# JvanKatwijk/sdr-j-fm

Measured on AMD Instinct MI355X. Metric: IQ MSamples/s demodulated to 48 kHz stereo, higher is better.
Workload: dtype f32 (stage A: 3-term split-f16 MFMA with a per-tile block exponent, f32 accumulate); 1 GPU; config4; population=established, channels_per_gpu=4096, channels_total=4096, streams_per_gpu=4096, block_samples_per_channel=230400, parallelism=channels sharded, 1 rank/GPU

## Files before the change

sdr-j-fm_amd/csrc/fmx_api.hip:

```cpp
#include "fmx_host.h"
#include "fmx_fftconv.h"
#include "fmx_design.h"

#include <cmath>
#include <cstdio>
#include <cstdlib>
#include <cstring>

thread_local std::string fmx::host::g_err;

namespace {

int env_int(const char *name, int dflt) { const char *v = getenv(name); return v ? atoi(v) : dflt; }
struct EnvSwitches {
    bool pieces_serial;
    bool tail_split;
};
const EnvSwitches &env_switches() {
    static const EnvSwitches sw{env_int("FMX_CALL_PIECES_SERIAL", 0) != 0, env_int("FMX_TAIL_SPLIT", 1) != 0};
    return sw;
}

int next_pow2(int64_t v) { int64_t p = 1; while (p < v) p <<= 1; return (int)p; }

int build_front_set(int32_t bw, int32_t inputRate, int32_t fmRate, int decim, int p, float *taps , FrontSet *fs) {
    std::vector<double> g(1, 1.0);
    double S1 = 0.0, S2 = 0.0;
    if (decim > 1) {
        const int32_t IRate = inputRate / 6;
        design::DecimKernel k1 = design::decim(4 * inputRate / IRate + 1, fmRate / 2, inputRate);
        design::DecimKernel k2 = design::decim(IRate / fmRate + 1, fmRate / 2, IRate);
        const int D1 = inputRate / IRate;
        g.assign((size_t)(D1 * (k2.hn.size() - 1) + k1.hn.size()), 0.0);
        for (size_t i = 0; i < k2.hn.size(); i++)
            for (size_t l = 0; l < k1.hn.size(); l++) g[D1 * i + l] += (double)k2.hn[i] * (double)k1.hn[l];
        S1 = k1.sum; S2 = k2.sum;
    }
    int L = 0;
    if (bw > 0) {
        std::vector<float> hin = design::lowpass(251, bw / 2, inputRate);
        g = design::convolve(g, design::to_double(hin));
        L = 2 * 32768 - 251;
    }
    const int NT = (int)g.size();
    const int64_t e = (int64_t)decim * p + decim - 1 - L;
    int64_t delay = -(e >= 0 ? e / 12 : -((-e + 11) / 12));
    const int off = (int)(e + 12 * delay);
    fs->off = off; fs->delay_fm = (int32_t)delay; fs->zshift = 0;
    int nd = 0;
    std::fill(taps, taps + A_TAPS_STRIDE, 0.f);
    for (int d = 0; d < A_MAX_ND; d++)
        for (int r = 0; r < DECIM; r++) {
            const int k = 12 * d + off - r;
            if (k >= 0 && k < NT) { taps[(d + 1) * DECIM + r] = (float)g[k]; nd = d + 1; }
        }
    fs->nd = nd;
    fs->gain_re = (float)(1.0 - S1 * S2); fs->gain_im = (float)(S1 + S2);
    double hs = 0, mk = 0;
    for (int d = 0; d < A_MAX_ND; d++)
        for (int r = 0; r < DECIM; r++) {
            const double v = (double)taps[(d + 1) * DECIM + r];
            hs += v; mk += v * (double)(12 * d + off - r);
        }
    fs->hsum = (float)hs;
    const double q0 = (double)off - mk / hs + 1.0;
    const int K = -(int)std::floor(q0 / 12.0);
    fs->dc_k = K; fs->dc_w = (float)((q0 + 12.0 * K) / 12.0);
    return (int)delay;
}

void build_audio_set(int32_t lf, int32_t fmRate, const std::vector<float> &rs, float *taps , AudioSet *as) {
    std::vector<double> g = design::to_double(rs);
    as->delay = 0;
    if (lf > 0) {
        std::vector<float> ha = design::lowpass(AUDIO_TAPS, lf, fmRate);
        g = design::convolve(design::to_double(ha), g);
        as->delay = AUDIO_DELAY;
    }
    as->ntaps = (int)g.size();
    std::fill(taps, taps + C_TAPS_STRIDE, 0.f);
    for (int kk = 0; kk < as->ntaps; kk++) taps[kk] = (float)g[as->ntaps - 1 - kk];
}

}

int fmx::host::ensure_sets(fmx_handle h) {
    std::vector<int32_t> fk, ak;
    for (int c = 0; c < h->channels; c++) {
        int32_t b = h->user[c].bw_applied, l = h->user[c].lf_applied > 0 ? h->user[c].lf_applied : 0;
        if (h->ola_mode) { b = 0; l = 0; }
        auto it = std::find(fk.begin(), fk.end(), b);
        if (it == fk.end()) { fk.push_back(b); it = fk.end() - 1; }
        h->params[c].front_set = (int)(it - fk.begin()) * h->twins;
        auto ia = std::find(ak.begin(), ak.end(), l);
        if (ia == ak.end()) { ak.push_back(l); ia = ak.end() - 1; }
        h->params[c].audio_set = (int)(ia - ak.begin());
    }
    if (fk != h->front_keys) {
        h->front_keys = fk;
        const size_t TW = (size_t)h->twins, NS = fk.size() * TW;
        h->h_front_taps.assign(NS * A_TAPS_STRIDE, 0.f);
        h->h_front_sets.resize(NS);
        for (size_t i = 0; i < fk.size(); i++) {
            int dmin = 0x7fffffff;
            std::vector<int> dl(TW);
            for (size_t p = 0; p < TW; p++) {
                dl[p] = build_front_set(fk[i], h->cfg.inputRate, h->cfg.fmRate, h->decim, (int)p, &h->h_front_taps[(i * TW + p) * A_TAPS_STRIDE], &h->h_front_sets[i * TW + p]);
                dmin = std::min(dmin, dl[p]);
            }
            for (size_t p = 0; p < TW; p++) { h->h_front_sets[i * TW + p].zshift = dl[p] - dmin; h->h_front_sets[i * TW + p].delay_fm = (int32_t)(TW * (size_t)dmin); }
        }
        if ((int)NS > h->front_cap) {
            h->mem.release(h->d_front_taps); h->mem.release(h->d_front_sets);
            h->front_cap = std::max<int>((int)NS, 4);
            FMXCHK(h->mem.alloc(h->d_front_taps, (size_t)A_TAPS_DEV * h->front_cap));
            FMXCHK(h->mem.alloc(h->d_front_sets, (size_t)h->front_cap));
        }
        HIPCHK(hipDeviceSynchronize());
        std::vector<float> dev(NS * A_TAPS_DEV, 0.f);
        for (size_t i = 0; i < NS; i++)
            for (int d = 0; d < A_MAX_ND; d++)
                for (int r = 0; r < DECIM; r++)
                    dev[i * A_TAPS_DEV + r * A_TAPS_ROW + d] = h->h_front_taps[i * A_TAPS_STRIDE + (d + 1) * DECIM + r];
        HIPCHK(hipMemcpy(h->d_front_taps, dev.data(), sizeof(float) * dev.size(), hipMemcpyHostToDevice));
        HIPCHK(hipMemcpy(h->d_front_sets, h->h_front_sets.data(), sizeof(FrontSet) * NS, hipMemcpyHostToDevice));
        h->T.front_taps = h->d_front_taps; h->T.front_sets = h->d_front_sets;
    }
    if (ak != h->audio_keys) {
        h->audio_keys = ak;
        h->h_audio_taps.assign(ak.size() * C_TAPS_STRIDE, 0.f);
        h->h_audio_sets.resize(ak.size());
        for (size_t i = 0; i < ak.size(); i++)
            build_audio_set(ak[i], h->cfg.fmRate, h->h_rs_taps, &h->h_audio_taps[i * C_TAPS_STRIDE], &h->h_audio_sets[i]);
        if ((int)ak.size() > h->audio_cap) {
            h->mem.release(h->d_audio_taps); h->mem.release(h->d_audio_sets);
            h->audio_cap = std::max<int>((int)ak.size(), 4);
            FMXCHK(h->mem.alloc(h->d_audio_taps, (size_t)C_TAPS_STRIDE * h->audio_cap));
            FMXCHK(h->mem.alloc(h->d_audio_sets, (size_t)h->audio_cap));
        }
        HIPCHK(hipDeviceSynchronize());
        HIPCHK(hipMemcpy(h->d_audio_taps, h->h_audio_taps.data(), sizeof(float) * h->h_audio_taps.size(), hipMemcpyHostToDevice));
        HIPCHK(hipMemcpy(h->d_audio_sets, h->h_audio_sets.data(), sizeof(AudioSet) * ak.size(), hipMemcpyHostToDevice));
        h->T.audio_taps = h->d_audio_taps; h->T.audio_sets = h->d_audio_sets;
        {
            std::vector<float> lp(ak.size() * AUDIO_TAPS, 0.f);
            for (size_t i = 0; i < ak.size(); i++) if (ak[i] > 0) { const std::vector<float> ha = design::lowpass(AUDIO_TAPS, ak[i], h->cfg.fmRate); std::copy(ha.begin(), ha.end(), lp.begin() + i * AUDIO_TAPS); }
            h->mem.release(h->T.audio_lp_taps);
            FMXCHK(h->mem.upload(h->T.audio_lp_taps, lp));
            if (!h->T.rs_taps) FMXCHK(h->mem.upload(h->T.rs_taps, h->h_rs_taps));
            std::vector<float2> W(fftc::W_COUNT), spec(ak.size() * 4 * fftc::N);
            fftc::make_twiddles(W.data());
            for (size_t i = 0; i < ak.size(); i++) {
                const int nt = h->h_audio_sets[i].ntaps;
                const float *rev = &h->h_audio_taps[i * C_TAPS_STRIDE];
                for (int p = 0; p < 4; p++) {
                    std::vector<float> gp;
                    for (int kk = p; kk < nt; kk += 4) gp.push_back(rev[nt - 1 - kk]);
                    fftc::make_spectrum(gp.data(), (int)gp.size(), &spec[(i * 4 + p) * fftc::N], W.data());
                }
            }
            h->mem.release(h->T.audio_spec);
            FMXCHK(h->mem.upload(h->T.audio_spec, spec));
        }
    }
    h->sets_dirty = false;
    return FMX_OK;
}

namespace {

void refresh_derived(fmx_handle h, int c) {
    const ChanUser &u = h->user[c];
    ChanParams &p = h->params[c];
    const int32_t fmRate = h->cfg.fmRate;
    if (u.deemph_us >= 1) {
        const float Tau = (float)(1000000.0 / u.deemph_us);
        p.deemph_alpha = (float)(1.0 / ((double)((float)fmRate / Tau) + 1.0));
    } else {
        p.deemph_alpha = (float)(1.0 / (fmRate / (1000000.0 / 50.0 + 1)));
    }
    p.deemph_l2 = (float)std::log2((double)(1.0f - p.deemph_alpha));
    p.volume = u.ctor_volume ? 0.5f : std::pow(10.0f, u.volume_db / 20.0f);
    p.left_ch = (u.balance > 0 ? (float)((100 - u.balance) / 100.0) : 1.0f);
    p.right_ch = (u.balance < 0 ? (float)((100 + u.balance) / 100.0) : 1.0f);
    p.panorama = (float)(int16_t)u.panorama / 100.0f;
}

int ensure_lo_table(fmx_handle h) {
    if (h->T.lo_table) return FMX_OK;
    const int32_t R = h->cfg.inputRate;
    std::vector<float2> tab((size_t)R);
    for (int32_t i = 0; i < R; i++)
        tab[i] = make_float2((float)std::cos(2.0 * design::kPi * i / R), (float)std::sin(2.0 * design::kPi * i / R));
    return h->mem.upload(h->T.lo_table, tab);
}

int ensure_rds_body(fmx_handle h);
int ensure_rds(fmx_handle h) {
    if (h->rds_alloc) return FMX_OK;
    const int rc = ensure_rds_body(h);
    if (rc) { h->rds_mem.release_all(); h->R = RdsBuffers{}; h->d_rds_nc0 = nullptr; h->rds_stage = nullptr; }
    return rc;
}
int ensure_rds_body(fmx_handle h) {
    const size_t C = (size_t)h->channels;
    const int32_t fmRate = h->cfg.fmRate;
    DevMem &M = h->rds_mem;
    RdsBuffers &R = h->R;
    FMXCHK(M.alloc(R.in_blk, C * RDS_BLK, true));
    FMXCHK(M.alloc(R.bpreal, C * 2 * RDS_BLK, true));
    FMXCHK(M.alloc(R.bp_over, 2 * C * 768, true));
    FMXCHK(M.alloc(R.hil, C * 2 * RDS_BLK, true));
    FMXCHK(M.alloc(R.hil_over, 2 * C * 768, true));
    FMXCHK(M.alloc(R.phase_ring, C * RDS_PHASE_RING, true));
    FMXCHK(M.alloc(R.U, C * 32768));
    FMXCHK(M.alloc(R.V, C * 32768));
    FMXCHK(M.alloc(R.rds24, C * RDS24_RING, true));
    R.pitch = h->pitch;
    FMXCHK(M.alloc(R.mf, (size_t)(h->work_nj / 8 + 8) * h->pitch));
    R.mfc_stride = ((h->work_nj / 8 + 8 + 2 + 7) / 8) * 8;
    FMXCHK(M.alloc(R.mfc, (size_t)R.mfc_stride * C, true));
    FMXCHK(M.alloc(R.mfm, (size_t)R.mfc_stride * C, true));
    FMXCHK(M.alloc(R.bits, C * RDS_BITS_CAP, true));
    FMXCHK(M.alloc(R.sym, C * RDS_SYM_CAP, true));
    {
        RdsState s0; std::memset(&s0, 0, sizeof(s0));
        s0.gain = 9.0f; s0.mu = 0.f; s0.skip = 3; s0.sample_count = 0;
        s0.c_limit = (float)(2 * design::kPi * (double)10.0f / (double)(float)24000);
        std::vector<RdsState> init(C, s0);
        FMXCHK(M.upload(R.state, init));
    }
    {
        const int N = 32768, D = 768;
        std::vector<float> k = design::bandpass(D, 3 * 19000 - 4800 / 2, 3 * 19000 + 4800 / 2, fmRate);
        std::vector<float2> S((size_t)N), Hm((size_t)N);
        std::vector<double> cs((size_t)N), sn((size_t)N);
        for (int i = 0; i < N; i++) { cs[i] = std::cos(-2 * design::kPi * i / N); sn[i] = std::sin(-2 * design::kPi * i / N); }
        for (int f = 0; f < N; f++) {
            double re = 0, im = 0;
            for (int i = 0; i < D; i++) {
                const int a = (int)(((int64_t)f * i) & (N - 1));
                re += (double)k[2 * i] * cs[a] - (double)k[2 * i + 1] * sn[a];
                im += (double)k[2 * i] * sn[a] + (double)k[2 * i + 1] * cs[a];
            }
            S[f] = make_float2((float)re, (float)im);
            Hm[f] = make_float2(f == 0 || f == N / 2 ? 1.0f : (f < N / 2 ? 2.0f : 0.0f), 0.f);
        }
        FMXCHK(M.upload(R.S_bp, S));
        FMXCHK(M.upload(R.S_hil, Hm));
        {
            std::vector<float2> Sr((size_t)N);
            for (int f = 0; f < N; f++) {
                const float2 a = S[(size_t)f], b = S[(size_t)((N - f) & (N - 1))];
                Sr[(size_t)f] = make_float2(0.5f * (a.x + b.x), 0.5f * (a.y - b.y));
            }
            FMXCHK(M.upload(R.S_bp_re, Sr));
        }
        std::vector<float> dk = design::decim_complex(11, 24000 / 2, fmRate);
        std::vector<float> rr = design::rrc(1.0, 24000, 2 * 1187.5f, 1.0, 45);
        float2 *dd;
        FMXCHK(M.alloc(dd, 11));
        FMXCHK(M.upload(R.rrc, rr));
        HIPCHK(hipMemcpy(dd, dk.data(), sizeof(float2) * 11, hipMemcpyHostToDevice));
        R.dec_taps = dd;
    }
    {
        FMXCHK(M.alloc(R.c_ring, C * RDS24_RING, true));
        FMXCHK(M.alloc(R.f_ring, C * RDS24_RING, true));
        FMXCHK(M.alloc(R.state1, C, true));
        std::vector<float> co = design::lowpass(RDS1_FIR, 2 * 2400, 24000);
        const std::vector<float> mk = design::rds1_match_kernel(24000);
        if ((int)mk.size() != RDS1_MATCH) return fail(FMX_E_HIP, "unexpected length of the RDS_1 matched filter");
        co.insert(co.end(), mk.begin(), mk.end());
        const design::Iir bp = design::iir_butterworth_bandpass(7, (int32_t)(1187.5 - 6), (int32_t)(1187.5 + 6), 24000);
        if (bp.nq != RDS1_QUADS) return fail(FMX_E_HIP, "unexpected biquad count of the RDS_1 band-pass");
        for (int i = 0; i < RDS1_QUADS; i++) { co.push_back(bp.q[i][1]); co.push_back(bp.q[i][2]); co.push_back(bp.q[i][4]); co.push_back(bp.q[i][5]); }
        co.push_back(bp.gain);
        FMXCHK(M.upload(R.rds1_coef, co));
        h->h_rds1 = co;
    }
    {
        FMXCHK(M.alloc(R.state3, C, true));
        std::vector<float2> sc24(24000);
        for (int i = 0; i < 24000; i++) sc24[i] = make_float2((float)std::cos(2 * design::kPi * i / 24000), (float)std::sin(2 * design::kPi * i / 24000));
        FMXCHK(M.upload(R.sincos24, sc24));
    }
    FMXCHK(M.alloc(R.sync, C, true));
    FMXCHK(M.alloc(R.groups, C * RDS_GROUP_RING, true));
    if (!h->ev_call) HIPCHK(hipEventCreateWithFlags(&h->ev_call, hipEventDisableTiming));
    h->rd.bits.assign(C, 0);
    {
        FMXCHK(M.alloc(h->d_rds_nc0, C, true));
        FMXCHK(M.alloc(R.chlist, C, true));
        R.nc0 = h->d_rds_nc0;
        h->rds_nc.assign(C, 0); h->rds_nc0.assign(C, -1); h->last_m0.assign(C, 0); h->last_m1.assign(C, 0);
    }
    h->rds_alloc = true;
    return FMX_OK;
}

int ola_alloc_side(fmx_handle h, fmx_handle_s::OlaSide &S, int L, int degree) {
    const size_t C = (size_t)h->channels;
    S.L = L; S.degree = degree;
    FMXCHK(h->mem.alloc(S.A, C * L, true));
    FMXCHK(h->mem.alloc(S.C, C * L, true));
    FMXCHK(h->mem.alloc(S.over, C * OLA_MAX_TAPS, true));
    FMXCHK(h->mem.alloc(S.over_new, C * OLA_MAX_TAPS, true));
    FMXCHK(h->mem.alloc(S.taps, C * OLA_MAX_TAPS, true));
    S.inp.assign(C, 0); S.on.assign(C, 0); S.key.assign(C, -1);
    return FMX_OK;
}
int ensure_ola(fmx_handle h) {
    if (h->d_v) return FMX_OK;
    const size_t C = (size_t)h->channels;
    FMXCHK(h->mem.alloc(h->d_v, C * h->cfg.max_block));
    FMXCHK(h->mem.alloc(h->d_u, C * h->cfg.max_block));
    FMXCHK(h->mem.alloc(h->d2ring, C * h->dring, true));
    h->pre_look.max_tiles = (int32_t)(h->cfg.max_block / PRE_TILE_SAMPLES + 1);
    FMXCHK(h->mem.alloc(h->pre_look.maps, C * h->pre_look.max_tiles));
    FMXCHK(h->mem.alloc(h->pre_look.flags, C * h->pre_look.max_tiles, true));
    FMXCHK(h->mem.alloc(h->pre_look.tickets, C, true));
    h->pre_look.ticket_base = 0;
// ... 352 lines not shown
    if (nd.prepass) { const int rc = ensure_prepass_arrays(h); if (rc) return rc; }
    for (int c = 0; c < h->channels; c++) {
        ChanUser &u = h->user[c];
        if (u.squelch_value != u.squelch_old) {
            u.squelch_level = u.squelch_value; u.squelch_old = u.squelch_value;
            const SquelchThr t = squelch_thresholds(u.squelch_level);
            h->params[c].squelch_thr = t.level; h->params[c].squelch_nthr = t.noise;
            h->params_dirty = true;
        }
    }
    if (h->params_dirty) {
        HIPCHK(hipDeviceSynchronize());
        HIPCHK(hipMemcpy(h->d_params, h->params.data(), sizeof(ChanParams) * h->channels, hipMemcpyHostToDevice));
        h->act_up.resize((size_t)h->channels);
        for (int c = 0; c < h->channels; c++) h->act_up[(size_t)c] = h->params[(size_t)c].actions;
        h->params_dirty = false;
    }
    return FMX_OK;
}

void actions_consumed(fmx_handle h, bool had_fm_samples) {
    std::lock_guard<std::mutex> lk(h->mtx);
    if (h->act_up.size() != (size_t)h->channels) return;
    const int32_t done = ACT_DC_RESET | (had_fm_samples ? (ACT_TRIGGER_FREQ | ACT_RESTART_PSS) : 0);
    for (int c = 0; c < h->channels; c++) {
        const int32_t clr = h->act_up[(size_t)c] & done;
        if (clr) { h->params[(size_t)c].actions &= ~clr; h->act_up[(size_t)c] &= ~clr; h->params_dirty = true; }
    }
}

void frames_geom(const fmx_handle h, int64_t n, CallGeom *G) {
    G->g0 = h->g_total; G->n = n;
    G->J0 = h->g_total / h->decim; G->J1 = (h->g_total + n) / h->decim;
    G->M0 = 48 * (G->J0 / 192); G->M1 = 48 * (G->J1 / 192);
}
int64_t call_frames(const fmx_handle h, int64_t n) { CallGeom G{}; frames_geom(h, n, &G); return conv2_out(h, G.M1) - conv2_out(h, G.M0); }

int ensure_pipe_streams(fmx_handle h) {
    if (h->pipe_sA) return FMX_OK;
    int lo = 0, hi = 0;
    HIPCHK(hipDeviceGetStreamPriorityRange(&lo, &hi));
    HIPCHK(hipStreamCreateWithPriority(&h->pipe_sA, hipStreamNonBlocking, lo));
    HIPCHK(hipStreamCreateWithPriority(&h->pipe_sB, hipStreamNonBlocking, lo));
    HIPCHK(hipStreamCreateWithPriority(&h->pipe_sP, hipStreamNonBlocking, hi));
    for (hipEvent_t *e : {&h->pipe_ev0, &h->pipe_evA, &h->pipe_evD, &h->pipe_evP, &h->pipe_evE, &h->pipe_evB[0], &h->pipe_evB[1]}) HIPCHK(hipEventCreateWithFlags(e, hipEventDisableTiming));
    return FMX_OK;
}

int check_call(fmx_handle h, int32_t fmt, float s16_den, int64_t n, int64_t pcm_stride) {
    if (const ParamCheck pc = check_iq_format(fmt, s16_den); pc.code) return fail(pc.code, pc.msg);
    if (n <= 0 || n > h->cfg.max_block) return fail(FMX_E_TOO_LARGE, "n_complex must be in [1, max_block]");
    if (call_frames(h, n) > pcm_stride) return fail(FMX_E_TOO_LARGE, "pcm_stride smaller than the frames this call produces");
    return FMX_OK;
}

struct CallArgs { int32_t fmt; float s16_den; int64_t stream_stride, pcm_stride; };

int promotion_turn(fmx_handle h, bool head, hipStream_t s, bool *capture) {
    bool do_promote = false, do_demote = false;
    {
        std::lock_guard<std::mutex> lk(h->mtx);
        if (h->ola_mode) {
            const bool ok = demotable(h);
            if (!ok || h->promo_recapture) { h->demo_capture = false; h->promo_have = 0; }
            else if (!h->demo_capture) { h->demo_capture = true; h->promo_have = 0; *capture = true; }
            else if (h->promo_have >= DEMO_TAIL_IN && head) do_demote = true;
            else *capture = true;
            h->promo_recapture = false;
        }
        else if (!h->promo_pending) h->promo_recapture = false;
        else if (h->promo_recapture) { h->promo_recapture = false; h->promo_have = 0; }
        else if (h->promo_have >= PROMO_TAIL_IN && head) do_promote = true;
        else *capture = true;
    }
    if (do_promote) return promote(h, s);
    if (do_demote) return demote(h, s);
    return FMX_OK;
}

int capture_samples(fmx_handle h, const void *d_iq, const CallArgs &a, const CallGeom &G, hipStream_t sa) {
    if (h->tail_iq && h->promo_have + G.n > h->tail_cap) return FMX_OK;
    if (!h->tail_iq) {
        h->tail_cap = PROMO_TAIL_IN + h->cfg.max_block;
        FMXCHK(h->mem.alloc(h->tail_iq, (size_t)h->streams * h->tail_cap));
        FMXCHK(h->mem.alloc(h->tail_snap, (size_t)h->channels));
    }
    if (h->promo_have == 0) { h->promo_g0 = h->g_total; launch_promo_state(h->B.state, h->tail_snap, h->channels, 0, sa); FMX_LAUNCHED(); }
    launch_capture(d_iq, a.fmt, G.iq_scale, a.stream_stride, G.n, h->streams, h->tail_iq, h->tail_cap, h->promo_have, sa); FMX_LAUNCHED();
    h->promo_have += G.n;
    return FMX_OK;
}

int stage_a(fmx_handle h, CallGeom &G, const void *d_iq, hipStream_t s, hipStream_t sa) {
    const FrontParts fp = plan_front_parts(G.g0, G.n, h->front_parts.load(), h->twins, h->channels, h->n_cus);
    if (fp.parts > 1 && !h->B.fsnap) {
        const size_t C = (size_t)h->channels;
        h->B.dc_pitch = (int32_t)(h->cfg.max_block / FRONT_TILE + 2);
        FMXCHK(h->mem.alloc(h->B.dc_tiles, 2 * (size_t)h->streams * h->B.dc_pitch));
        FMXCHK(h->mem.alloc(h->B.fsnap, C));
        FMXCHK(h->mem.alloc(h->B.hist_snap, C * DECIM * A_HIST_COLS));
        FMXCHK(h->mem.alloc(h->B.dcv_snap, C * DCV_SAVE));
    }
    const FrontChoice fc = choose_front(h->needs.front4_ok, h->needs.any_lo, h->front_kernel.load(), fp.parts, h->channels, h->n_cus);
    G.parts = fc.parts; G.part_tiles = fp.part_tiles; G.front4 = fc.front4;
    h->last_front_kernel = (G.front4 && front4_tiles(G, d_iq) > 0) ? 3 : 1;
    if (h->ola_mode) {
        if (const int rc = ola_input_side(h, G, h->B, d_iq, s)) return rc;
        CallGeom Gp = G; Gp.pre_processed = 1; Gp.iq_format = 0; Gp.iq_scale = 1.0f; Gp.stream_stride = h->cfg.max_block; Gp.streams_private = h->twins == 1 ? 1 : 0;
        launch_front(h->T, h->B, Gp, h->d_u, h->channels, s);
    } else
    launch_front(h->T, h->B, G, d_iq, h->channels, sa);
    FMX_LAUNCHED();
    return FMX_OK;
}

int stage_b(fmx_handle h, const CallGeom &G, int k, bool piped, int second, hipStream_t s, hipStream_t sa) {
    if (piped) {
        HIPCHK(hipEventRecord(h->pipe_evA, sa)); HIPCHK(hipStreamWaitEvent(s, h->pipe_evA, 0));
        if (k >= 2) HIPCHK(hipStreamWaitEvent(sa, h->pipe_evB[k & 1], 0));
        DeviceBuffers Bk = h->B;
        if (k & 1) { const size_t off = (size_t)prepass_half(h->work_nj) * (size_t)h->pitch; Bk.w_iq += off; Bk.w_osc += off; }
        const PrepassStreams ps{sa, h->pipe_sP, h->pipe_evD, h->pipe_evP};
        launch_demod_fused(h->T, Bk, G, h->channels, s, &ps);
        HIPCHK(hipEventRecord(h->pipe_evB[k & 1], s));
    } else if (second > 0) {
        HIPCHK(hipEventRecord(h->pipe_evA, s)); HIPCHK(hipStreamWaitEvent(h->pipe_sA, h->pipe_evA, 0));
        CallGeom G1 = G, G2 = G;
        G1.ch0 = 0; G1.ch_count = h->channels - second; G2.ch0 = h->channels - second; G2.ch_count = second;
        launch_demod_fused(h->T, h->B, G1, h->channels, s);
        launch_demod_fused(h->T, h->B, G2, h->channels, h->pipe_sA);
    } else
    launch_demod_fused(h->T, h->B, G, h->channels, s);
    if (G.J1 > G.J0) {
        int cnt = h->my_count_host + (int)(G.J1 - G.J0);
        if (cnt > (SINCOS_N >> 1)) cnt -= (SINCOS_N >> 1) + 1;
        h->my_count_host = cnt;
    }
    return FMX_OK;
}

int stage_rds(fmx_handle h, const CallGeom &G, hipStream_t s) {
    const int64_t nj = G.J1 - G.J0;
    int modes = 0;
    for (int c = 0; c < h->channels; c++) {
        const int m = h->call_rds_mode[(size_t)c];
        modes |= 1 << m;
        h->rds_nc0[(size_t)c] = m != 0 ? h->rds_nc[(size_t)c] : -1;
    }
    HIPCHK(hipMemcpyAsync(h->d_rds_nc0, h->rds_nc0.data(), sizeof(int64_t) * (size_t)h->channels, hipMemcpyHostToDevice, s));
    launch_rds(h->B, h->R, G, h->channels, h->rds_nc0.data(), modes, s);
    for (int c = 0; c < h->channels; c++) {
        const int64_t a = h->rds_nc0[(size_t)c];
        if (a < 0) { h->last_m0[(size_t)c] = h->last_m1[(size_t)c]; continue; }
        h->last_m0[(size_t)c] = a / 8; h->last_m1[(size_t)c] = (a + nj) / 8;
        h->rds_nc[(size_t)c] = a + nj;
    }
    return FMX_OK;
}

int stage_scan(fmx_handle h, const CallGeom &G, hipStream_t sa) {
    const int64_t nj = G.J1 - G.J0;
    const size_t n = h->call_scan.size();
    h->scan_jobs.resize(n);
    {
        std::lock_guard<std::mutex> lk(h->mtx);
        for (size_t i = 0; i < n; i++) {
            const int c = h->call_scan[i];
            const ScanProduce sp = scan_produce(h->scan_fill[(size_t)c], h->scan_blocks[(size_t)c], nj, G.J0, scan::N, scan::RING);
            h->scan_jobs[i] = ScanJob{c, sp.job_fill, sp.job_slot0, 0};
            for (int64_t b = sp.b0; b < sp.nblk; b++) {
                const size_t slot = (size_t)c * scan::RING + (size_t)sp.slot(b);
                h->scan_end[slot] = sp.end_sample(b);
                h->scan_rec_thr[slot] = h->call_scan_thr[i];
            }
            h->scan_blocks[(size_t)c] = sp.new_blocks;
            h->scan_fill[(size_t)c] = sp.new_fill;
        }
    }
    HIPCHK(hipMemcpyAsync(h->d_scan_jobs, h->scan_jobs.data(), sizeof(ScanJob) * n, hipMemcpyHostToDevice, sa));
    ScanArgs A{};
    A.jobs = h->d_scan_jobs; A.zring = h->B.zring; A.params = h->d_params; A.front_sets = h->d_front_sets; A.W = h->d_scan_W;
    A.carry = h->d_scan_carry; A.rec = h->d_scan_rec; A.J0 = G.J0; A.J1 = G.J1; A.ring_mask = G.ring_mask;
    launch_scan(A, (int)n, sa); FMX_LAUNCHED();
    return FMX_OK;
}

int stage_meter(fmx_handle h, const CallGeom &G, hipStream_t s) {
    const int64_t nj = G.J1 - G.J0;
    if (nj > h->work_nj) return fail(FMX_E_TOO_LARGE, "the piece has more fm samples than stage B's rows hold");
    h->meter_jobs.clear();
    {
        std::lock_guard<std::mutex> lk(h->mtx);
        for (int c = 0; c < h->channels; c++) {
            if (!h->call_meter[(size_t)c]) { h->meter_on_from[(size_t)c] = -1; continue; }
            if (h->meter_on_from[(size_t)c] < 0) h->meter_on_from[(size_t)c] = G.J0;
            const meter::Produce mp = meter::meter_produce(h->meter_on_from[(size_t)c], G.J0, nj, h->meter_produced[(size_t)c]);
            if (mp.first >= G.J1) continue;
            h->meter_jobs.push_back(MeterJob{c, (int32_t)(mp.first - G.J0), (int32_t)mp.slot(0), 0});
            h->meter_produced[(size_t)c] = mp.new_produced;
        }
    }
    const size_t n = h->meter_jobs.size();
    if (n == 0) return FMX_OK;
    HIPCHK(hipMemcpyAsync(h->d_meter_jobs, h->meter_jobs.data(), sizeof(MeterJob) * n, hipMemcpyHostToDevice, s));
    MeterArgs A{};
    A.jobs = h->d_meter_jobs; A.w_dem = h->B.w_dem; A.w_cur = h->B.w_cur; A.state = h->d_meter_state; A.ring = h->d_meter_ring;
    A.J0 = G.J0; A.J1 = G.J1; A.lin_rows = h->B.lin_rows;
    launch_meter(A, (int)n, s); FMX_LAUNCHED();
    return FMX_OK;
}

int stage_scan_mute(fmx_handle h, float2 *d_pcm, int64_t pcm_stride, int64_t frames, hipStream_t s) {
    const size_t n = h->call_scan.size();
    HIPCHK(hipMemcpyAsync(h->d_scan_mute, h->call_scan.data(), sizeof(int32_t) * n, hipMemcpyHostToDevice, s));
    launch_scan_mute(h->d_scan_mute, (int)n, d_pcm, pcm_stride, frames, s); FMX_LAUNCHED();
    return FMX_OK;
}

int stage_audio_meter(fmx_handle h, const CallGeom &G, const float2 *d_pcm, int64_t frames, hipStream_t s) {
    h->loud_jobs.clear();
    {
        std::lock_guard<std::mutex> lk(h->mtx);
        for (int c = 0; c < h->channels; c++) {
            if (!h->call_loud[(size_t)c]) { h->loud_on_from[(size_t)c] = -1; continue; }
            if (h->loud_on_from[(size_t)c] < 0) h->loud_on_from[(size_t)c] = G.M0;
            const loud::Produce ap = loud::audio_produce(h->loud_on_from[(size_t)c], G.M0, frames, h->loud_produced[(size_t)c]);
            h->loud_jobs.push_back(LoudJob{c, ap.first == G.M0 ? 1 : 0, (int32_t)ap.slot(0), ap.reset ? 1 : 0});
            h->loud_produced[(size_t)c] = ap.new_produced;
        }
    }
    const size_t n = h->loud_jobs.size();
    if (n == 0) return FMX_OK;
    HIPCHK(hipMemcpyAsync(h->d_loud_jobs, h->loud_jobs.data(), sizeof(LoudJob) * n, hipMemcpyHostToDevice, s));
    LoudArgs A{};
    A.jobs = h->d_loud_jobs; A.pcm = d_pcm; A.pcm_stride = G.pcm_stride; A.state = h->d_loud_state; A.ring = h->d_loud_ring;
    A.M0 = G.M0; A.frames = (int32_t)frames;
    launch_loud(A, (int)n, s); FMX_LAUNCHED();
    return FMX_OK;
}

int stage_c(fmx_handle h, CallGeom &G, float2 *d_pcm, int64_t frames, int second, hipStream_t s) {
    DeviceBuffers Bq = h->B;
    if (h->ola_mode && G.J1 > G.J0) {
        OlaBuffers O{}; O.src = h->B.dring; O.dst = h->d2ring; O.src_stride = O.dst_stride = h->dring; O.src_mask = O.dst_mask = h->dring - 1;
        O.src_pos = O.dst_pos = G.J0;
        HStep st1;
        if (ola_single_step(h, h->ola_au, G.J1 - G.J0, &st1)) {
            OlaStepRef ref; const int rc = step_ref(h, st1, s, &ref); if (rc) return rc;
            ola_fill(h->ola_au, O);
            launch_deemph(h->B, G, h->d2ring, h->channels, s, &ref, &O); FMX_LAUNCHED();
            ola_finish_single(h, h->ola_au, st1, ref, O, s);
        } else {
            const int rc = run_ola(h, h->ola_au, O, G.J1 - G.J0, s); if (rc) return rc;
            launch_deemph(h->B, G, h->d2ring, h->channels, s, nullptr, nullptr); FMX_LAUNCHED();
        }
    }
    if (h->ola_mode) Bq.dring = h->d2ring;
    if (h->gain_pending && G.M1 > G.M0) { G.gain_fix = 1; launch_gain_fix(h->T, Bq, G, h->channels, s); FMX_LAUNCHED(); h->gain_pending = false; }
    if (second > 0) {
        CallGeom G1 = G, G2 = G;
        G1.ch0 = 0; G2.ch0 = h->channels - second;
        launch_audio(h->T, Bq, G1, d_pcm, h->channels - second, s);
        launch_audio(h->T, Bq, G2, d_pcm, second, h->pipe_sA);
        HIPCHK(hipEventRecord(h->pipe_evE, h->pipe_sA)); HIPCHK(hipStreamWaitEvent(s, h->pipe_evE, 0));
    } else if (!h->cv_nt) launch_audio(h->T, Bq, G, d_pcm, h->channels, s);
    else {
        CallGeom G48 = G; G48.pcm_stride = h->x48_stride;
        launch_audio(h->T, Bq, G48, h->d_x48 + h->cv_nt, h->channels, s);
        launch_conv2(h->d_x48, h->x48_stride, h->d_cv_taps, h->cv_p, h->cv_q, h->cv_nt, G.M0, G.M1 - G.M0, conv2_out(h, G.M0), frames,
                     d_pcm, G.pcm_stride, h->channels, s);
    }
    return FMX_OK;
}

int run_piece(fmx_handle h, const CallArgs &a, const void *d_iq, int64_t n, float2 *d_pcm, hipStream_t s, int k, bool overlapped, int64_t *n_frames) {
    bool capture = false;
    int rc = promotion_turn(h, k == 0, s, &capture);
    if (rc || (rc = flush_mailbox(h))) return rc;
    CallGeom G{};
    frames_geom(h, n, &G);
    G.ring_mask = h->ring - 1; G.dring_mask = h->dring - 1; G.sring_mask = h->sring - 1;
    G.input_rate = h->cfg.inputRate; G.pitch = h->pitch; G.streams_private = (h->streams_private && h->twins == 1) ? 1 : 0; G.twins = h->twins; G.channels = h->channels; G.stream_stride = a.stream_stride; G.pcm_stride = a.pcm_stride;
    G.iq_format = a.fmt; G.iq_scale = (a.fmt == 3) ? 1.0f / a.s16_den : 1.0f / 128.0f; G.n_cus = h->n_cus; G.streams = h->streams;
    const int64_t frames = conv2_out(h, G.M1) - conv2_out(h, G.M0);
    const bool rds_running = h->rds_alloc && h->needs.any_rds;
    if (rds_running && G.J1 - G.J0 > RDS_BLK)
        return fail(FMX_E_TOO_LARGE, "with RDS on, a call may cover at most 32000 fm samples (384000 input samples)");
    const bool piped = overlapped && !h->ola_mode && !env_switches().pieces_serial;
    hipStream_t sa = piped ? h->pipe_sA : s;
    G.host_count1 = piped ? h->my_count_host + 1 : 0;
    ProfRec pr{}; const bool prof = h->prof_on;
    if (prof) {
        for (int i = 0; i < 4; i++) HIPCHK(hipEventCreate(&pr.e[i]));
        pr.in_samples = n * h->streams; pr.ch_samples = n * h->channels;
        HIPCHK(hipEventRecord(pr.e[0], sa));
    }
    g_launch_err = hipSuccess;
    h->B.lin_rows = (int32_t)h->work_nj;
    if (capture && (rc = capture_samples(h, d_iq, a, G, sa))) return rc;
    if ((rc = stage_a(h, G, d_iq, s, sa))) return rc;
    if (!h->call_scan.empty() && G.J1 > G.J0 && (rc = stage_scan(h, G, sa))) return rc;
    if (prof) HIPCHK(hipEventRecord(pr.e[1], sa));
    G.stageb_form = h->stageb_form.load(); G.no_deemph = h->ola_mode ? 1 : 0;
    const bool plain = plain_batch(PieceFlags{piped, h->ola_mode, h->B.w_iq != nullptr, h->cv_nt != 0, h->needs.rows_on, rds_running, h->gain_pending, G.stageb_form,
                                              G.J1 > G.J0, G.M1 > G.M0});
    const int second = env_switches().tail_split && plain ? second_group_channels(h->channels, h->n_cus) : 0;
    if (second > 0 && (rc = ensure_pipe_streams(h))) return rc;
    h->last_second_group = second;
    if ((rc = stage_b(h, G, k, piped, second, s, sa))) return rc;
    if (rds_running && (rc = stage_rds(h, G, s))) return rc;
    if (h->meter_alloc && G.J1 > G.J0 && (rc = stage_meter(h, G, s))) return rc;
    if (prof) HIPCHK(hipEventRecord(pr.e[2], s));
    if ((rc = stage_c(h, G, d_pcm, frames, second, s))) return rc;
    if (!h->call_scan.empty() && frames > 0 && (rc = stage_scan_mute(h, d_pcm, G.pcm_stride, frames, s))) return rc;
    if (h->loud_alloc && frames > 0 && (rc = stage_audio_meter(h, G, d_pcm, frames, s))) return rc;
    if (prof) { HIPCHK(hipEventRecord(pr.e[3], s)); h->prof.push_back(pr); }
    FMX_LAUNCHED();
    HIPCHK(g_launch_err);
    actions_consumed(h, G.J1 > G.J0);
    h->last_J0 = G.J0; h->last_J1 = G.J1;
    h->g_total += n;
    if (n_frames) *n_frames = frames;
    return FMX_OK;
}

int run_call(fmx_handle h, const void *d_iq, int32_t fmt, float s16_den, int64_t stream_stride, int64_t n, float2 *d_pcm,
             int64_t pcm_stride, int64_t *n_frames, hipStream_t s) {
    h->last_pieces = 1;
    int rc = check_call(h, fmt, s16_den, n, pcm_stride);
    if (rc) return rc;
    CallShape cs{};
    {
        std::lock_guard<std::mutex> lk(h->mtx);
        const CallNeeds nd = summarize(h);
        cs.any_rds = nd.any_rds; cs.prepass = nd.prepass; cs.pllc = nd.pllc; cs.am = nd.am;
    }
    if (!cs.any_rds && cs.prepass && !h->ola_mode && (rc = ensure_prepass_arrays(h))) return rc;
    cs.n = n; cs.decim = h->decim; cs.call_pieces = h->pipe_rows.load(); cs.channels = h->channels; cs.ola_mode = h->ola_mode; cs.conv2 = h->cv_nt != 0;
    cs.prepass_arrays = h->B.w_iq != nullptr; cs.half = prepass_half(h->work_nj);
    const CallPlan plan = plan_call(cs);
    const bool overlapped = plan.kind == CallKind::OVERLAPPED;
    hipStream_t ps = s;
    if (overlapped) {
        if ((rc = ensure_pipe_streams(h))) return rc;
        HIPCHK(hipEventRecord(h->pipe_ev0, s));
        HIPCHK(hipStreamWaitEvent(h->pipe_sA, h->pipe_ev0, 0)); HIPCHK(hipStreamWaitEvent(h->pipe_sB, h->pipe_ev0, 0));
        ps = h->pipe_sB;
    }
    const CallArgs a{fmt, s16_den, stream_stride, pcm_stride};
    const int64_t bps = bytes_per_sample(fmt);
    int64_t pos = 0, total = 0;
    for (size_t k = 0; k < plan.lens.size(); k++) {
        int64_t got = 0;
        rc = run_piece(h, a, reinterpret_cast<const char *>(d_iq) + pos * bps, plan.lens[k], d_pcm + total, ps, (int)k, overlapped, &got);
        if (rc) { if (overlapped) (void)hipDeviceSynchronize(); return rc; }
        pos += plan.lens[k]; total += got;
    }
    if (overlapped) {
        HIPCHK(hipEventRecord(h->pipe_evE, h->pipe_sB)); HIPCHK(hipStreamWaitEvent(s, h->pipe_evE, 0));
        h->last_pieces = (int)plan.lens.size();
    }
    if (h->rds_alloc) { HIPCHK(hipEventRecord(h->ev_call, s)); h->ev_call_set = true; }
    if (n_frames) *n_frames = total;
    return FMX_OK;
}


}

namespace {

struct Conv2Design { int p = 1, q = 1, nt = 0; std::vector<float> taps; };

int validate_config(const fmx_config *cfg, int *decim_out, Conv2Design *cv) {
    if (cfg->struct_size != (int32_t)sizeof(fmx_config)) return fail(FMX_E_INVALID, "fmx_config.struct_size mismatch");
    if (cfg->channels < 1) return fail(FMX_E_INVALID, "channels must be >= 1");
    if (cfg->fmRate != 192000 || cfg->workingRate != 48000)
        return fail(FMX_E_UNSUPPORTED, "this build implements fmRate 192000 / workingRate 48000 (radio.cpp:68,231-233)");
    int decim = DECIM;
    {
        if (cfg->inputRate < 1 || cfg->inputRate > 100000000) return fail(FMX_E_INVALID, "inputRate out of range");
        if (cfg->inputRate / cfg->fmRate <= 1) decim = 1;
        else {
            const int32_t IRate = cfg->inputRate / 6;
            const int64_t d2 = IRate / cfg->fmRate;
            if ((d2 != 1 && d2 != 2) || 4 * (int64_t)cfg->inputRate / IRate + 1 != 25 || cfg->inputRate / IRate != 6)
                return fail(FMX_E_UNSUPPORTED, "inputRate: built are the rates the reference decimates by 12 (2304000 <= inputRate < 3456000), by 6 "
                                               "(1152000 <= inputRate < 2304000) and not at all (inputRate < 384000); below 1152000 the reference's "
                                               "second decimator has one tap and a zero gain (fir-filters.cpp:327-347), from 3456000 on it divides by 3+");
            decim = 6 * (int)d2;
        }
    }
    *decim_out = decim;
    if (cfg->audioRate != cfg->workingRate) {
        if (cfg->audioRate < 8000 || cfg->audioRate > 192000 ||
            !design::design_conv2(cfg->workingRate, cfg->audioRate, &cv->p, &cv->q, &cv->nt, &cv->taps))
            return fail(FMX_E_UNSUPPORTED, "audioRate: 8000 .. 192000 with audioRate / gcd (audioRate, workingRate) <= 640 (the second converter's phases)");
    }
    if (cfg->max_block < 12 || cfg->max_block > (1 << 20)) return fail(FMX_E_INVALID, "max_block must be in [12, 1048576]");
    int ndev = 0;
    if (hipGetDeviceCount(&ndev) != hipSuccess || ndev <= 0)
        return fail(FMX_E_NO_DEVICE, "no HIP device visible: libfmx has no CPU fallback");
    if (cfg->device < 0 || cfg->device >= ndev) return fail(FMX_E_INVALID, "device ordinal out of range");
    return FMX_OK;
}

int init_channels(fmx_handle h, const fmx_config *cfg, int decim, const Conv2Design &cv) {
    h->cfg = *cfg; h->cfg.stream_of_channel = nullptr;
    h->decim = decim; h->twins = DECIM / decim;
    h->channels = cfg->channels;
    h->streams = cfg->streams > 0 ? cfg->streams : cfg->channels;
    if (cv.nt) {
        h->cv_p = cv.p; h->cv_q = cv.q; h->cv_nt = cv.nt;
        h->x48_stride = cv.nt + cfg->max_block / (4 * h->decim) + 96;
    }
    h->ola_mode = filter_form(0, h->channels).ola_mode;
    h->user.assign(h->channels, ChanUser());
    h->rd.init((size_t)h->channels);
    h->params.assign(h->channels, ChanParams());
    for (int c = 0; c < h->channels; c++) {
        ChanParams &p = h->params[c];
        std::memset(&p, 0, sizeof(p));
        int s = cfg->stream_of_channel ? cfg->stream_of_channel[c] : (cfg->streams > 0 ? c % h->streams : c);
        if (s < 0 || s >= h->streams) return fail(FMX_E_INVALID, "stream_of_channel entry out of range");
        p.stream = s;
        p.fm_mode = 0; p.sound_sel = 0; p.decoder = 3; p.auto_mono = 1; p.pss_active = 1; p.dc_remove = 1;
        p.rds_mode = 0; p.lo_freq = 0; p.lo_period = 0; p.att_l = 1.f; p.att_r = 1.f;
        p.pll_seq = pll_seq(0, h->channels);
        const SquelchThr t = squelch_thresholds(1);
        p.squelch_mode = 0; p.squelch_thr = t.level; p.squelch_nthr = t.noise;
        refresh_derived(h, c);
    }
    std::vector<int> users((size_t)h->streams, 0);
    h->streams_private = true;
    for (auto &p : h->params) if (++users[(size_t)p.stream] > 1) h->streams_private = false;
    return FMX_OK;
}

int init_device(fmx_handle h) {
    hipDeviceProp_t dp;
    HIPCHK(hipGetDeviceProperties(&dp, h->cfg.device));
    h->n_cus = dp.multiProcessorCount;
    int optin = 0;
    if (hipDeviceGetAttribute(&optin, hipDeviceAttributeMaxSharedMemoryPerBlock, h->cfg.device) != hipSuccess) optin = 0;
    h->lds_per_block = std::max((size_t)dp.sharedMemPerBlock, (size_t)optin);
    HIPCHK(hipStreamCreateWithFlags(&h->stream, hipStreamNonBlocking));
    HIPCHK(hipEventCreateWithFlags(&h->ev_in, hipEventDisableTiming));
    return FMX_OK;
}

int build_trig_tables(fmx_handle h) {
    const int32_t fmRate = h->cfg.fmRate;
    std::vector<float2> sc((size_t)SINCOS_N);
    for (int i = 0; i < SINCOS_N; i++)
        sc[i] = make_float2((float)std::cos(2 * design::kPi * i / fmRate), (float)std::sin(2 * design::kPi * i / fmRate));
    FMXCHK(h->mem.upload(h->T.sincos, sc));
    {
        SinPoly sp{}; sp.step = 2 * design::kPi / fmRate;
        bool fits = (fmRate == SINCOS_N);
        for (int i = 0; fits && i < SINCOS_N; i++) {
            float sn, cs;
            sincos_poly(i, sp.step, &sn, &cs);
            if (std::memcmp(&sn, &sc[i].y, 4) != 0) { if (sp.ns < 4) { sp.s_idx[sp.ns] = i; sp.s_val[sp.ns] = sc[i].y; sp.ns++; } else fits = false; }
            if (std::memcmp(&cs, &sc[i].x, 4) != 0) { if (sp.nc < 4) { sp.c_idx[sp.nc] = i; sp.c_val[sp.nc] = sc[i].x; sp.nc++; } else fits = false; }
        }
        sp.ok = fits ? 1 : 0;
        h->T.sp = sp;
    }
    {
        std::vector<double2> tr((size_t)TRIG2_N);
        for (int a = 0; a < TRIG2_A; a++) { double t = 2 * design::kPi * (256.0 * a) / fmRate; tr[a] = make_double2(std::cos(t), std::sin(t)); }
        for (int a = 0; a < TRIG2_APAD; a++) tr[TRIG2_A + a] = tr[a];
        for (int b = 0; b < TRIG2_B; b++) { double t = 2 * design::kPi * (double)b / fmRate; tr[TRIG2_A + TRIG2_APAD + b] = make_double2(std::cos(t), std::sin(t)); }
        bool exact = (fmRate == TRIG2_A * TRIG2_B);
        for (int i = 0; exact && i < SINCOS_N; i++) {
            const double2 ea = tr[i >> 8], eb = tr[TRIG2_A + TRIG2_APAD + (i & 255)];
            const float sn = (float)(ea.y * eb.x + ea.x * eb.y);
            if (std::memcmp(&sn, &sc[i].y, 4) != 0) exact = false;
        }
        if (exact) FMXCHK(h->mem.upload(h->T.trig2, tr));
    }
    {
        const float P32 = 6.2831855f;
        const float C32 = (float)((double)P32 - 2 * design::kPi);
        bool ok = true;
        for (float v = P32; ok && v < P32 + 0.7f; v = std::nextafterf(v, 100.f)) {
            const float want = (float)((double)v - 2 * design::kPi);
            volatile float d = v - P32;
            const float got = d + C32;
            if (std::memcmp(&want, &got, 4) != 0) ok = false;
        }
        h->T.wrap32_c = C32; h->T.wrap32_ok = ok ? 1 : 0;
    }
    std::vector<float> at((size_t)ATAN_N + 1);
    const float St = (float)design::kPi;
    for (int i = 0; i <= ATAN_N; i++) { float f = (float)i / ATAN_N; at[i] = (float)((double)(std::atan(f) * St) / design::kPi); }
    FMXCHK(h->mem.upload(h->T.atan_ppy, at));
    std::vector<float> as((size_t)ARCSINE_N + 1);
    for (int i = 0; i <= ARCSINE_N; i++) as[i] = (float)(std::asin(2.0 * i / ARCSINE_N - 1.0) / 2.0);
    return h->mem.upload(h->T.arcsine, as);
}

int build_filter_tables(fmx_handle h) {
    const int32_t fmRate = h->cfg.fmRate;
    h->h_pss_taps = design::lowpass(PSS_TAPS, 15000, fmRate);
    FMXCHK(h->mem.upload(h->T.pss_taps, h->h_pss_taps));
    h->h_rs_taps = design::resampler(RS_TAPS);
    {
        std::vector<float2> W(fftc::W_COUNT), Hs(fftc::N);
        fftc::make_twiddles(W.data());
        fftc::make_spectrum(h->h_pss_taps.data(), PSS_TAPS, Hs.data(), W.data());
        FMXCHK(h->mem.upload(h->T.fft_w, W));
        FMXCHK(h->mem.upload(h->T.pss_hs, Hs));
    }
    h->T.sincos_C = fmRate / (2 * design::kPi);
    {
        const float F_G = (float)(0.65 * fmRate / 2), Delta_F = (float)(0.95 * fmRate / 2);
        const float B_FM = 2 * (Delta_F + F_G);
        h->T.K_FM = (float)((double)(2 * B_FM) * design::kPi / (double)F_G);
        const float max_dev = (float)(0.95 * (0.5 * fmRate));
        const float fac = (float)(2.0 * design::kPi / fmRate);
        h->T.pll_beta = (float)std::exp(-2.0 * design::kPi * (double)(float)(0.85 * fmRate) / 2 / fmRate);
        h->T.pll_lo = -max_dev * fac; h->T.pll_hi = max_dev * fac; h->T.pll_center = (float)(0 * 2 * design::kPi / fmRate);
    }
    h->T.pil_omega = (float)((double)((float)19000 / (float)fmRate) * (2 * design::kPi));
    h->T.pil_gain = (float)(10 * (2 * design::kPi) / fmRate);
    h->T.K_FM_rcp = 1.0f / h->T.K_FM; h->T.pil_omega_rcp = 1.0f / h->T.pil_omega;
    h->T.pss_alpha = 10.0f / (float)fmRate;
    h->T.pss_lock_alpha = 1.0f / fmRate;
    h->T.afc_l2 = (float)std::log2((double)(1 - 0.0001f));
    h->T.lock_l2 = (float)std::log2(1.0 - (double)(1.0f / 3000.0f));
    h->T.pssmean_l2 = (float)std::log2((double)(1.0f - h->T.pss_lock_alpha));
    return FMX_OK;
}

int alloc_channel_buffers(fmx_handle h, const Conv2Design &cv) {
    DevMem &M = h->mem;
    DeviceBuffers &B = h->B;
    const int32_t max_block = h->cfg.max_block;
    const int64_t fm_per_call = max_block / h->decim + 2;
    h->ring = next_pow2((2 * 32768 - 251) / h->decim + 1 + fm_per_call + 512);
    h->dring = next_pow2(std::max<int64_t>(AUDIO_DELAY + C_MAX_TAPS, h->channels > OLA_MAX_CH ? PROMO_TAIL_AU + 8 : 0) + fm_per_call + 192 + 4 * C_TILE);
    h->sring = 4096;
    const size_t C = (size_t)h->channels;
    const size_t CT = C * (size_t)h->twins;
    if (cv.nt) {
        FMXCHK(M.upload(h->d_cv_taps, cv.taps));
        FMXCHK(M.alloc(h->d_x48, C * h->x48_stride, true));
    }
    FMXCHK(M.alloc(B.hist, CT * DECIM * A_HIST_COLS, true));
    FMXCHK(M.alloc(B.dcv_hist, CT * DCV_SAVE, true));
    if (h->twins > 1) FMXCHK(M.alloc(B.state_tw, C * (size_t)(h->twins - 1), true));
    FMXCHK(M.alloc(B.zring, C * h->ring, true));
    FMXCHK(M.alloc(B.sring, C * h->sring, true));
    FMXCHK(M.alloc(B.dring, C * h->dring, true));
    {
        const size_t NJ = (((size_t)fm_per_call + 1 + WT - 1) / WT) * WT;
        h->work_nj = (int64_t)NJ;
        h->pitch = ((h->channels + 63) / 64) * 64 + 64;
        const size_t P = (size_t)h->pitch;
        FMXCHK(M.alloc(B.w_dem, NJ * P, true));
        FMXCHK(M.alloc(B.w_cur, NJ * P, true));
        B.lockm_stride = (int32_t)(NJ / 6 + 512);
        FMXCHK(M.alloc(B.w_lockm, (size_t)B.lockm_stride * P, true));
        FMXCHK(M.alloc(B.gfix, GAIN_FIX_FRAMES * P, true));
    }
    {
        ChanState s0; std::memset(&s0, 0, sizeof(s0));
        s0.Imin1 = s0.Qmin1 = s0.Imin2 = s0.Qmin2 = (float)0.01;
        FMXCHK(M.upload(B.state, std::vector<ChanState>(C, s0)));
    }
    FMXCHK(M.alloc(h->d_params, C));
    B.params = h->d_params;
    {
        std::vector<float> tone((size_t)TT_BURST);
        float ph = 0.0f; const float inc = (float)(2 * design::kPi / h->cfg.workingRate * 1000.0f);
        for (int i = 0; i < TT_BURST; i++) {
            ph += inc;
            if (!(0 <= ph && ph < 2 * design::kPi)) ph = (float)std::fmod((double)ph, 2 * design::kPi);
            tone[i] = std::sin(ph);
        }
        FMXCHK(M.upload(B.tone, tone));
        B.pk_tiles = (int32_t)((max_block / (4 * h->decim) + 96) / C_TILE + 8);
        FMXCHK(M.alloc(B.pk_part, C * B.pk_tiles, true));
        FMXCHK(M.alloc(B.pk_ring, C * PK_RING, true));
    }
    return FMX_OK;
}

}

extern "C" {

int fmx_abi_version(void) { return FMX_ABI_VERSION; }
const char *fmx_last_error(void) { return g_err.c_str(); }

int fmx_create(const fmx_config *cfg, fmx_handle *out) {
    if (!cfg || !out) return fail(FMX_E_INVALID, "null argument");
    (void)env_switches();
    int decim = DECIM;
    Conv2Design cv;
    FMXCHK(validate_config(cfg, &decim, &cv));
    HIPCHK(hipSetDevice(cfg->device));

    fmx_handle h = new (std::nothrow) fmx_handle_s();
    if (!h) return fail(FMX_E_NOMEM, "out of host memory");
// ... 203 lines not shown
```

sdr-j-fm_amd/csrc/fmx_internal.h:

```cpp
#pragma once
#include <hip/hip_runtime.h>
#include <stdint.h>
#include "fmx_plan.h"
#include "fmx_needs.h"
#include "fmx_rdssync.h"

namespace fmx {

constexpr int A_TILE_COLS = 256;
constexpr int A_HIST_COLS = 25;
constexpr int A_MAX_ND = 25;
constexpr int A_TAPS_STRIDE = (A_MAX_ND + 2) * DECIM;
constexpr int A_TAPS_ROW = 32;
constexpr int A_TAPS_DEV = DECIM * A_TAPS_ROW;
constexpr int PSS_TAPS = 295;
constexpr int PSS_DELAY = 2048 - 295;
constexpr int PSS_CHUNK = 1744;
constexpr int RS_TAPS = 128;
constexpr int AUDIO_TAPS = 756;
constexpr int AUDIO_DELAY = 8192 - 756;
constexpr int C_MAX_TAPS = AUDIO_TAPS + RS_TAPS - 1;
constexpr int C_TAPS_STRIDE = 896;
constexpr int C_TILE = 256;
constexpr int GAIN_FIX_BACK = RS_TAPS + 192;
constexpr int GAIN_FIX_FRAMES = GAIN_FIX_BACK / 4;
constexpr int NSQ_QUADS = 10;
constexpr int TT_SILENT = 96001;
constexpr int TT_BURST = 1200;
constexpr int TT_CYCLE = TT_SILENT + TT_BURST;
constexpr int PK_WIN = 961;
constexpr int PK_RING = 256;
constexpr int SINCOS_N = 192000;
constexpr int ATAN_N = 8192;
constexpr int ARCSINE_N = 4 * 8192;
constexpr int TRIG2_A = 750, TRIG2_B = 256;
constexpr int TRIG2_APAD = 2;
constexpr int TRIG2_N = TRIG2_A + TRIG2_APAD + TRIG2_B;

struct FrontSet {
    int32_t nd;
    int32_t off;
    int32_t delay_fm;
    float   gain_re, gain_im;
    float   hsum, dc_w;
    int32_t dc_k;
    int32_t zshift;
};
constexpr int DCV_SAVE = 16;

struct AudioSet {
    int32_t ntaps;
    int32_t delay;
};

struct ChanParams {
    int32_t stream;
    int32_t front_set, audio_set;
    int32_t fm_mode, sound_sel, decoder, auto_mono, pss_active, dc_remove, rds_mode;
    int32_t lo_freq;
    int32_t lo_period;
    float   att_l, att_r;
    float   deemph_alpha, volume, left_ch, right_ch, panorama;
    int32_t actions;
    int32_t squelch_mode;
    float   squelch_thr;
    int32_t test_tone;
    float   squelch_nthr;
    float   deemph_l2;
    float   hlo_re, hlo_im;
    int32_t pll_seq;
};
enum { ACT_TRIGGER_FREQ = 1, ACT_RESTART_PSS = 2, ACT_DC_RESET = 4 };

struct ChanState {
    float   dc_re, dc_im;
    int32_t lo_phase;
    float   Imin1, Qmin1, Imin2, Qmin2, fm_afc, am_carr;
    float   nco_phase, phase_incr;
    float   pil_phase, pil_old, pil_lock;
    int32_t pil_stable, pil_locked;
    float   pss_acc, pss_mean;
    int32_t pss_lock_cnt, pss_unlock_cnt, pss_minimized;
    float   pilot_delay_pss;
    int64_t pss_count;
    int32_t pss_call_total;
    int32_t pad0;
    float   de_l, de_r;
    float   prev_gl, prev_gr;
    int32_t gain_valid, pad_g;
    int64_t fade_start_frame;
    int32_t my_count;
    float   meta_dc_rf, meta_dc_if, meta_pss_deg, meta_pss_change, meta_lock_strength;
    int32_t meta_pss_state, meta_locked;
    int32_t sq_count, sq_suppress;
    int32_t tt_pos;
    int32_t pk_cnt;
    float   pk_l, pk_r;
    int32_t pk_events;
    int32_t hist_fmt;
    float   sq_avg_hi, sq_avg_lo;
    float   sq_m[2][NSQ_QUADS][2];
    int32_t pll_replays;
    int32_t pll_newton_ok;
    int32_t pll_exact_segs, pad_x;
};

constexpr int WT = 16;
__host__ __device__ __forceinline__ size_t widx(int64_t r, int ch, int pitch) {
    return ((size_t)(r >> 4) * (size_t)pitch + (size_t)ch) * WT + (size_t)(r & 15);
}

struct SinPoly {
    double step;
    int32_t ok, ns, nc, pad_;
    int32_t s_idx[4]; float s_val[4];
    int32_t c_idx[4]; float c_val[4];
};
__host__ __device__ __forceinline__ void sincos_poly(int idx, double step, float *sn, float *cs) {
    constexpr int OCT = SINCOS_N / 8;
    const int q = idx / OCT, r = idx - OCT * q, k = q & 3;
    const int rr = (k & 1) ? OCT - r : r;
    const double x = (double)rr * step, z = x * x;
    double ps = -1.0 / 1307674368000.0;
    ps = __builtin_fma(ps, z, 1.0 / 6227020800.0); ps = __builtin_fma(ps, z, -1.0 / 39916800); ps = __builtin_fma(ps, z, 1.0 / 362880);
    ps = __builtin_fma(ps, z, -1.0 / 5040); ps = __builtin_fma(ps, z, 1.0 / 120); ps = __builtin_fma(ps, z, -1.0 / 6);
    const double sv = __builtin_fma(x * z, ps, x);
    double pc = 1.0 / 20922789888000.0;
    pc = __builtin_fma(pc, z, -1.0 / 87178291200.0); pc = __builtin_fma(pc, z, 1.0 / 479001600); pc = __builtin_fma(pc, z, -1.0 / 3628800);
    pc = __builtin_fma(pc, z, 1.0 / 40320); pc = __builtin_fma(pc, z, -1.0 / 720); pc = __builtin_fma(pc, z, 1.0 / 24); pc = __builtin_fma(pc, z, -0.5);
    const double cv = __builtin_fma(z, pc, 1.0);
    double s, c;
    switch (k) {
    default:
    case 0: s = sv; c = cv; break;
    case 1: s = cv; c = sv; break;
    case 2: s = cv; c = -sv; break;
    case 3: s = sv; c = -cv; break;
    }
    if (q >= 4) { s = -s; c = -c; }
    *sn = (float)s; *cs = (float)c;
}

struct DeviceTables {
    const float2 *sincos;
    const float  *atan_ppy;
    const float  *arcsine;
    const float2 *lo_table;
    const double2 *trig2;
    const float  *front_taps;
    const FrontSet *front_sets;
    const float  *pss_taps;
    const float2 *fft_w;
    const float2 *pss_hs;
    const float  *audio_taps;
    const float  *audio_lp_taps;
    const float  *rs_taps;
    const float2 *audio_spec;
    const AudioSet *audio_sets;
    double  sincos_C;
    float   K_FM, K_FM_rcp, pil_omega_rcp;
    float   pil_omega, pil_gain, pss_alpha, pss_lock_alpha;
    float   afc_l2, lock_l2, pssmean_l2;
    float   pll_beta, pll_lo, pll_hi, pll_center;
    const float *nsq_coef;
    SinPoly sp;
    float   wrap32_c;
    int32_t wrap32_ok;
};

struct CallGeom {
    int64_t g0;
    int64_t n;
    int64_t J0, J1;
    int64_t M0, M1;
    int32_t ring_mask;
    int32_t dring_mask;
    int32_t sring_mask;
    int32_t input_rate;
    int32_t pitch;
    int32_t streams_private;
    int64_t stream_stride, pcm_stride;
    int32_t iq_format;
    float   iq_scale;
    int32_t gain_fix;
    int32_t stageb_form;
    int32_t twins;
    int32_t channels;
    int32_t n_cus;
    int32_t pre_processed;
    int32_t no_deemph;
    int32_t streams;
    int32_t front4;
    int32_t cont;
    int32_t ch_count;
    int32_t ch0;
    int32_t host_count1;
    int32_t parts, part_tiles;
};
struct FrontSnap { int32_t lo_phase, hist_fmt; float dc_re, dc_im; };

constexpr int DBG_SLOTS = 96;
struct DeviceBuffers {
    float2 *hist;
    float2 *dcv_hist;
    float2 *zring;
    float2 *sring;
    float2 *dring;
    ChanState *state;
    ChanState *state_tw;
    const ChanParams *params;
    unsigned long long *dbg;
    float   *w_dem;
    float   *w_cur;
    float   *w_diff;
    float2  *w_iq;
    float   *w_osc;
    float2  *gfix;
    uint8_t *w_lockm;
    int32_t lockm_stride;
    int32_t prepass;
    int32_t peaks_on;
    int32_t rows_on;
    int32_t prepass_var;
    const float *tone;
    float4  *pk_part;
    float2  *pk_ring;
    int32_t pk_tiles;
    int32_t lin_rows;
    float4  *dc_tiles;
    int32_t dc_pitch;
    FrontSnap *fsnap;
    float2  *hist_snap;
    float2  *dcv_snap;
};
__host__ __device__ __forceinline__ size_t tap_idx(const DeviceBuffers &B, int64_t r, int ch, int pitch) {
    return B.lin_rows ? (size_t)ch * (size_t)B.lin_rows + (size_t)r : widx(r, ch, pitch);
}

constexpr int OLA_MAX_TAPS = 768;
struct OlaChan { int32_t off, len, inp; int16_t on, conv; };
struct OlaStep { OlaChan ch[OLA_MAX_CH]; };
struct OlaStepRef { OlaStep val; const OlaChan *tab; };
struct OlaBuffers {
    const float2 *src; float2 *dst;
    int64_t src_stride, dst_stride, src_mask, dst_mask, src_pos, dst_pos;
    float2 *A, *C;
    float2 *over, *over_new;
    const float *taps;
    int32_t L, degree;
};
struct PreLook { float4 *maps; int32_t *flags; int32_t max_tiles, epoch; uint32_t *tickets; uint32_t ticket_base; };
constexpr int PRE_TILE_SAMPLES = 8192;
void launch_pre(const DeviceTables &T, const DeviceBuffers &B, const CallGeom &G, const void *iq, float2 *vbuf, int64_t vstride, int channels, hipStream_t s,
                const OlaStepRef *S, const OlaBuffers *O, const PreLook &LB);
void launch_ola_io(const OlaStepRef &S, const OlaBuffers &O, int channels, int maxlen, hipStream_t s);
void launch_ola_conv(const OlaStepRef &S, const OlaBuffers &O, int channels, hipStream_t s);
void launch_deemph(const DeviceBuffers &B, const CallGeom &G, float2 *ring, int channels, hipStream_t s, const OlaStepRef *S, const OlaBuffers *O);

constexpr int PROMO_TAIL_IN = 3 * (2 * 32768 - 251) + 1024;
constexpr int PROMO_TAIL_AU = 3 * (2 * 4096 - AUDIO_TAPS) + 1200;
constexpr int64_t DEMO_QUIET = 3 * (2 * 32768 - 251) + 4096;
constexpr int DEMO_TAIL_IN = (2 * 32768 - 251) + 4096;
constexpr int DEMO_TAIL_AU = AUDIO_DELAY + C_MAX_TAPS + 2048;
void launch_capture(const void *iq, int fmt, float qs, int64_t stream_stride, int64_t n, int streams, float2 *tail, int64_t tail_cap, int64_t pos, hipStream_t s);
void launch_promo_state(ChanState *st, FrontSnap *snap, int channels, int mode, hipStream_t s);
void launch_promo_hist(float2 *hist, const float2 *u, int64_t u_stride, int64_t len, int r0, int twins, float2 *zring, int ring_mask, int64_t J0,
                       const ChanParams *params, const FrontSet *old_sets, const int32_t *old_set_of, int channels, hipStream_t s);
void launch_promo_inv_deemph(const float2 *dring, int dmask, int64_t J0, int NA, const ChanParams *params, float2 *out, int channels, hipStream_t s);

constexpr int RDS_PHASE_RING = 131072;
constexpr int RDS24_RING = 8192;
constexpr int RDS_BITS_CAP = 8192;
constexpr int RDS_SYM_CAP = 1024;
struct RdsState {
    float gain, mu, c_freq, c_phase, c_limit;
    int32_t sample_count, skip, prev_bit, nbits;
    float2 sb0, sb1, sb2;
};
constexpr int RDS1_FIR = 21, RDS1_MATCH = 43, RDS1_QUADS = 8;
struct Rds1State {
    float c_freq, c_phase;
    float m1[RDS1_QUADS], m2[RDS1_QUADS];
    float last_sync_slope, last_sync, last_data;
    int32_t prev_bit;
};
struct Rds3State {
    float c_freq, c_phase;
    float bit_integrator, bit_clk_phase, prev_clk_state;
    int32_t prev_bit, resync_pending, started;
    uint32_t bs_stream; int32_t bs_synced, bs_cur, bs_bits_in_blk, bs_sync_err, bs_blk1;
};
struct RdsBuffers {
    float  *in_blk;
    float  *bpreal;
    float2 *bp_over;
    float2 *hil;
    float2 *hil_over;
    float  *phase_ring;
    float2 *U, *V;
    float2 *rds24;
    float2 *mf;
    float2 *mfc;
    float  *mfm;
    int64_t mfc_stride;
    RdsState *state;
    uint8_t *bits;
    float2 *sym;
    const float2 *S_bp, *S_hil;
    const float2 *S_bp_re;
    const float2 *dec_taps;
    const float *rrc;
    float  *c_ring, *f_ring;
    Rds1State *state1;
    const float *rds1_coef;
    Rds3State *state3;
    const float2 *sincos24;
    int32_t pitch;
    const int64_t *nc0;
    int *chlist;
    RdsSyncChan *sync;
    RdsGroupRec *groups;
};
#define C_RDS_PITCH(Rb) ((Rb).pitch)
void launch_rds(const DeviceBuffers &B, const RdsBuffers &Rb, const CallGeom &G, int C, const int64_t *h_nc0, int modes, hipStream_t s);

struct ScanJob { int32_t ch, fill, slot0, pad; };
struct ScanArgs {
    const ScanJob *jobs;
    const float2 *zring;
    const ChanParams *params; const FrontSet *front_sets;
    const float2 *W;
    float2 *carry;
    float2 *rec;
    int64_t J0, J1;
    int32_t ring_mask, pad;
};
void launch_scan(const ScanArgs &A, int n_jobs, hipStream_t s);
void launch_scan_mute(const int32_t *chans, int n, float2 *pcm, int64_t pcm_stride, int64_t frames, hipStream_t s);

struct MeterJob { int32_t ch, r0, slot0, pad; };
struct MeterArgs {
    const MeterJob *jobs;
    const float *w_dem, *w_cur;
    float *state;
    fmx_mod_record *ring;
    int64_t J0, J1;
    int32_t lin_rows, pad;
};
void launch_meter(const MeterArgs &A, int n_jobs, hipStream_t s);

struct LoudJob { int32_t ch, acc, slot0, reset; };
struct LoudArgs {
    const LoudJob *jobs;
    const float2 *pcm;
    int64_t pcm_stride;
    float *state;
    fmx_audio_record *ring;
    int64_t M0;
    int32_t frames, pad;
};
void launch_loud(const LoudArgs &A, int n_jobs, hipStream_t s);

constexpr int W_RATE0 = 2304000;
constexpr int W_MIN_K = 2, W_MAX_K = 16;
constexpr int W_HCOLS = 16;
constexpr int W_HIST = W_HCOLS * W_MAX_K;
constexpr int W_TILE = 256;
constexpr int W_MAX_SEG = 17;
struct WideSeg { int64_t nbase; int32_t pbase, f; };
struct WideOut { int32_t stream, nseg; WideSeg seg[W_MAX_SEG]; };
struct WideArgs {
    const void *src; int32_t fmt; float qs;
    int64_t src_stride, n_wide, n_out, g0;
    float2 *dst; int64_t dst_stride;
    const float2 *hist_in; float2 *hist_out;
    const float2 *taps;
    const float *h;
    const float2 *rot;
    const WideOut *outs;
    const int32_t *first, *list;
};
void launch_wide(const WideArgs &A, int K, int streams, hipStream_t s);

struct WideRateArgs {
    const void *src; int32_t fmt; float qs;
    int64_t src_stride, n_wide, n_out, g0, j0;
    float2 *dst; int64_t dst_stride;
    const float2 *hist_in; float2 *hist_out;
    int32_t Rw, L, M, NP;
    const float *phases;
    const float2 *rot;
    const WideOut *outs;
    const int32_t *first, *list;
};
void launch_wide_rate(const WideRateArgs &A, int streams, hipStream_t s);

struct SurveyArgs {
    const void *src; int32_t fmt; float qs;
    int64_t src_stride, n_wide;
    int64_t blocks;
    int32_t fill, fill_after;
    int32_t phase, B, slot0, fresh;
    float scale;
    int64_t power_stride;
    const float *window; const float2 *W;
    float2 *carry;
    float *power;
    float *acc;
    float *ring;
};
void launch_survey(const SurveyArgs &A, int streams, hipStream_t s);

void launch_front(const DeviceTables &T, const DeviceBuffers &B, const CallGeom &G, const void *iq,
                  int channels, hipStream_t s);
int front4_tiles(const CallGeom &G, const void *iq);
void launch_front4(const DeviceTables &T, const DeviceBuffers &B, const CallGeom &G, const void *iq, int channels, hipStream_t s);
void launch_front4_lo(const DeviceTables &T, const DeviceBuffers &B, const CallGeom &G, const void *iq, int channels, hipStream_t s);
extern thread_local hipError_t g_launch_err;
inline void note_hip(hipError_t e) { if (e != hipSuccess && g_launch_err == hipSuccess) g_launch_err = e; }
#define FMX_LAUNCHED() ::fmx::note_hip(hipGetLastError())
struct PrepassStreams { hipStream_t s_disc, s_afc; hipEvent_t ev_disc, ev_afc; };
void launch_demod_prepass(const DeviceTables &T, const DeviceBuffers &B, const CallGeom &G, int channels, hipStream_t s, const PrepassStreams *ps = nullptr);
void launch_demod_fused(const DeviceTables &T, const DeviceBuffers &B, const CallGeom &G, int channels, hipStream_t s, const PrepassStreams *ps = nullptr);
void launch_audio(const DeviceTables &T, const DeviceBuffers &B, const CallGeom &G, float2 *pcm,
                  int channels, hipStream_t s);
void launch_conv2(float2 *x48, int64_t x_stride, const float *taps, int p, int q, int nt, int64_t in0, int64_t frames_in,
                  int64_t out0, int64_t nout, float2 *pcm, int64_t pcm_stride, int channels, hipStream_t s);
void launch_gain_fix(const DeviceTables &T, const DeviceBuffers &B, const CallGeom &G, int channels, hipStream_t s);

}
```

sdr-j-fm_amd/csrc/fmx_plan.h:

```cpp
#pragma once
#include <cstdint>
#include <vector>

namespace fmx {

constexpr int DECIM = 12;
constexpr int RDS_BLK = 32000;
constexpr int STAGEB_SEG = 1536;
constexpr int STAGEB_WG_PER_CU = 3;

constexpr int PIPE_ROWS_AUTO = 3072;
constexpr int PIPE_ROWS_AUTO_PLL = 4608;
constexpr int PIPE_ROWS_AUTO_AM = 3840;
constexpr int PIPE_ROWS_AUTO_SQ = 4608;
constexpr int PIPE_MIN_CHANNELS = 1024;
constexpr int TAIL_MIN_CHANNELS = 128;

inline int64_t prepass_half(int64_t work_nj) { return (work_nj / 2) & ~(int64_t)15; }

struct CallShape {
    int64_t n; int decim;
    bool any_rds;
    bool prepass, pllc, am;
    int call_pieces, channels;
    bool ola_mode, conv2, prepass_arrays;
    int64_t half;
};
enum class CallKind { WHOLE, RDS_PIECES, OVERLAPPED };
struct CallPlan { CallKind kind; std::vector<int64_t> lens; };

inline CallPlan plan_call(const CallShape &c) {
    const int64_t n = c.n, d = c.decim;
    if (c.any_rds) {
        const int64_t piece = (int64_t)(RDS_BLK - 1) * d;
        if (n <= piece) return {CallKind::WHOLE, {n}};
        CallPlan p{CallKind::RDS_PIECES, {}};
        for (int64_t pos = 0; pos < n; pos += piece) p.lens.push_back(n - pos < piece ? n - pos : piece);
        return p;
    }
    const int want = c.call_pieces;
    const int64_t auto_rows = c.am ? PIPE_ROWS_AUTO_AM : PIPE_ROWS_AUTO_PLL;
    const int64_t rows = want > 0 ? ((want + 15) / 16) * 16 : (c.pllc ? (n < 2 * auto_rows * d ? PIPE_ROWS_AUTO : auto_rows) : PIPE_ROWS_AUTO_SQ);
    const int64_t piece = rows * d;
    if (!(c.prepass && c.prepass_arrays && want != 0 && !c.ola_mode && !c.conv2 && (want > 0 || c.channels >= PIPE_MIN_CHANNELS) && rows + 2 <= c.half && n >= 2 * piece))
        return {CallKind::WHOLE, {n}};
    CallPlan p{CallKind::OVERLAPPED, {}};
    if (want < 0 && c.pllc) {
        const int64_t seg = (int64_t)STAGEB_SEG * d;
        int64_t pos = 0;
        while (n - pos >= 2 * piece) { p.lens.push_back(piece); pos += piece; }
        const int64_t R = n - pos;
        int64_t a = ((R - seg) / (seg / 2)) * (seg / 2);
        if (a > piece) a = piece;
        if (a >= seg) { p.lens.push_back(a); p.lens.push_back(R - a); } else p.lens.push_back(R);
        bool fits = true;
        for (int64_t l : p.lens) fits = fits && l > 0 && l / d + 2 <= c.half;
        if (fits) return p;
        p.lens.clear();
    }
    for (int64_t pos = 0; pos < n;) {
        int64_t len = (n - pos < piece) ? n - pos : piece;
        if (n - pos - len > 0 && n - pos - len < piece / 2 && (rows * 3) / 2 + 2 <= c.half) len = n - pos;
        p.lens.push_back(len); pos += len;
    }
    return p;
}

constexpr int FRONT_MIN_PART_TILES = 6, FRONT_MAX_PARTS = 32, FRONT_TILE = 128 * DECIM;
struct FrontParts { int parts, part_tiles; };
inline FrontParts plan_front_parts(int64_t g0, int64_t n, int want, int twins, int channels, int n_cus) {
    const FrontParts one{1, 0};
    if (twins != 1 || want == 1) return one;
    const int64_t r0 = g0 % DECIM;
    const int NT = (int)((r0 + n - 1) / FRONT_TILE) + 1;
    int parts = want > 1 ? want : (2 * n_cus) / channels;
    if (want <= 1 && parts > NT / FRONT_MIN_PART_TILES) parts = NT / FRONT_MIN_PART_TILES;
    if (parts > FRONT_MAX_PARTS) parts = FRONT_MAX_PARTS;
    if (parts > NT / 2) parts = NT / 2;
    if (parts < 2) return one;
    const int pt = (NT + parts - 1) / parts;
    parts = (NT + pt - 1) / pt;
    if (parts < 2) return one;
    return {parts, pt};
}

inline bool stageb_two_kernels(int channels, int n_cus, bool rows_on, int form, int wg_per_cu) {
    if (form) return form == 2;
    const int cus = n_cus > 0 ? n_cus : 256;
    const long whole = (long)((channels + wg_per_cu * cus - 1) / (wg_per_cu * cus)) * wg_per_cu * 100;
    const long halves = (long)((channels + 4 * cus - 1) / (4 * cus)) * 4 * 102;
    return rows_on && halves < whole;
}

inline int second_group_channels(int channels, int n_cus) {
    const int slots = STAGEB_WG_PER_CU * (n_cus > 0 ? n_cus : 256);
    if (channels <= slots) return 0;
    int first_rounds = (int)(0.65 * (double)channels / (double)slots + 0.5);
    if (first_rounds < 1) first_rounds = 1;
    const int tail = channels - first_rounds * slots;
    return tail < TAIL_MIN_CHANNELS ? 0 : tail;
}

}
```

sdr-j-fm_amd/csrc/fmx_stageb.hip:

```cpp
#include "fmx_internal.h"
#include "fmx_demod_math.h"
#include "fmx_fftconv.h"
#include <type_traits>

namespace fmx {

#define SB_TICK(k) do { if (dbg_on) { const unsigned long long now_ = clock64(); dbg_acc[k] += now_ - dbg_t; dbg_t = now_; } } while (0)
#ifdef SB_FINE_TICKS
#define SB_FT(k) do { if (ft_on) { const unsigned long long now_ = clock64(); atomicAdd(&ft_acc[k], now_ - ft_t); ft_t = now_; } } while (0)
#define SB_FTW(k) do { asm volatile("s_waitcnt vmcnt(0) lgkmcnt(0)" ::: "memory"); SB_FT(k); } while (0)
#else
#define SB_FT(k) do { } while (0)
#define SB_FTW(k) do { } while (0)
#endif

constexpr int FB_T = 256, FB_W = STAGEB_SEG, FB_K = FB_W / FB_T;
static_assert(FB_K * FB_T == FB_W, "a thread's samples tile the segment");
static_assert(FB_T == fftc::T, "the convolution is written for the workgroup size");
static_assert(FB_W <= PSS_DELAY, "a segment's PSS errors must only need s-ring entries of earlier segments");
constexpr int PSS_MAX_ROUNDS = 64;
#ifndef SB_WG_PER_SIMD
#define SB_WG_PER_SIMD STAGEB_WG_PER_CU
#endif

template <int CTRL, int RM> __device__ __forceinline__ int dppi(int old, int v) { return __builtin_amdgcn_update_dpp(old, v, CTRL, RM, 0xf, false); }
template <int CTRL> __device__ __forceinline__ int dppzi(int v) { return __builtin_amdgcn_mov_dpp(v, CTRL, 0xf, 0xf, true); }
template <int CTRL> __device__ __forceinline__ float dppzf(float v) { return __int_as_float(dppzi<CTRL>(__float_as_int(v))); }
template <int CTRL> __device__ __forceinline__ double dppzd(double v) { return __hiloint2double(dppzi<CTRL>(__double2hiint(v)), dppzi<CTRL>(__double2loint(v))); }
template <int CTRL, int RM> __device__ __forceinline__ float dppf(float old, float v) { return __int_as_float(dppi<CTRL, RM>(__float_as_int(old), __float_as_int(v))); }
template <int CTRL, int RM> __device__ __forceinline__ double dppd(double old, double v) {
    const int lo = dppi<CTRL, RM>(__double2loint(old), __double2loint(v));
    const int hi = dppi<CTRL, RM>(__double2hiint(old), __double2hiint(v));
    return __hiloint2double(hi, lo);
}
__device__ __forceinline__ double wscan_add_d(double v) {
    v += dppzd<0x111>(v); v += dppzd<0x112>(v); v += dppzd<0x114>(v); v += dppzd<0x118>(v);
    v += dppd<0x142, 0xa>(0.0, v); v += dppd<0x143, 0xc>(0.0, v);
    return v;
}
__device__ __forceinline__ float wscan_add_f(float v) {
    v += dppzf<0x111>(v); v += dppzf<0x112>(v); v += dppzf<0x114>(v); v += dppzf<0x118>(v);
    v += dppf<0x142, 0xa>(0.f, v); v += dppf<0x143, 0xc>(0.f, v);
    return v;
}
__device__ __forceinline__ int wscan_add_i(int v) {
    v += dppzi<0x111>(v); v += dppzi<0x112>(v); v += dppzi<0x114>(v); v += dppzi<0x118>(v);
    v += dppi<0x142, 0xa>(0, v); v += dppi<0x143, 0xc>(0, v);
    return v;
}
constexpr int IMIN = -0x7fffffff - 1;
__device__ __forceinline__ int imax(int a, int b) { return a > b ? a : b; }
__device__ __forceinline__ int wscan_max_i(int v) {
    v = imax(v, dppi<0x111, 0xf>(IMIN, v)); v = imax(v, dppi<0x112, 0xf>(IMIN, v)); v = imax(v, dppi<0x114, 0xf>(IMIN, v));
    v = imax(v, dppi<0x118, 0xf>(IMIN, v)); v = imax(v, dppi<0x142, 0xa>(IMIN, v)); v = imax(v, dppi<0x143, 0xc>(IMIN, v));
    return v;
}
__device__ __forceinline__ float lane_prev_f(float v, float id) { return dppf<0x138, 0xf>(id, v); }
__device__ __forceinline__ int lane_prev_i(int v, int id) { return dppi<0x138, 0xf>(id, v); }
__device__ __forceinline__ double lane_prev_d(double v, double id) { return dppd<0x138, 0xf>(id, v); }

__device__ __forceinline__ double powi(double b, int n) { double r = 1.0; while (n) { if (n & 1) r *= b; b *= b; n >>= 1; } return r; }

struct DecayW { float m1, m2, m4, m8, mA, mB, dl, d64; };
__device__ __forceinline__ DecayW make_decay(float l2, int lane) {
    DecayW w;
    const float L = l2 * (float)FB_K;
    w.m1 = __builtin_amdgcn_exp2f(L); w.m2 = __builtin_amdgcn_exp2f(2 * L); w.m4 = __builtin_amdgcn_exp2f(4 * L); w.m8 = __builtin_amdgcn_exp2f(8 * L);
    w.mA = __builtin_amdgcn_exp2f((float)((lane & 15) + 1) * L); w.mB = __builtin_amdgcn_exp2f((float)((lane & 31) + 1) * L);
    w.dl = __builtin_amdgcn_exp2f((float)lane * L); w.d64 = __builtin_amdgcn_exp2f(64 * L);
    return w;
}
enum { DEC_AFC = 0, DEC_LOCK = 1, DEC_PSSMEAN = 2, DEC_DEEMPH = 3 };
template <int NSCANS> struct DecayTab { float4 w[NSCANS][64][2]; };
template <int NSCANS> __device__ __forceinline__ void store_decay(DecayTab<NSCANS> *tab, int which, float l2, int lane) {
    const DecayW w = make_decay(l2, lane);
    tab->w[which % NSCANS][lane][0] = make_float4(w.m1, w.m2, w.m4, w.m8);
    tab->w[which % NSCANS][lane][1] = make_float4(w.mA, w.mB, w.dl, w.d64);
}
template <int NSCANS> __device__ __forceinline__ DecayW load_decay(const DecayTab<NSCANS> *tab, int which, int lane) {
    const float4 a = tab->w[which % NSCANS][lane][0], b = tab->w[which % NSCANS][lane][1];
    DecayW w; w.m1 = a.x; w.m2 = a.y; w.m4 = a.z; w.m8 = a.w; w.mA = b.x; w.mB = b.y; w.dl = b.z; w.d64 = b.w;
    return w;
}
__device__ __forceinline__ float wscan_decay(float v, const DecayW &w) {
    v = fmaf(dppzf<0x111>(v), w.m1, v); v = fmaf(dppzf<0x112>(v), w.m2, v);
    v = fmaf(dppzf<0x114>(v), w.m4, v); v = fmaf(dppzf<0x118>(v), w.m8, v);
    v = fmaf(dppf<0x142, 0xa>(0.f, v), w.mA, v); v = fmaf(dppf<0x143, 0xc>(0.f, v), w.mB, v);
    return v;
}

struct ScanLds {
    double wd[2][4][2];
    float  wf[2][4][4];
    int    wi[2][4][4];
    float  edge[FB_T];
};



struct WG {
    ScanLds *L; int tid, lane, wv, sl;
    __device__ __forceinline__ float decay_incoming(float Lt, float Y0, const DecayW &w) {
        const float Z = wscan_decay(Lt, w);
        if (lane == 63) L->wf[sl][wv][0] = Z;
        __syncthreads();
        float C = Y0;
        for (int v = 0; v < wv; v++) C = fmaf(C, w.d64, L->wf[sl][v][0]);
        sl ^= 1;
        return fmaf(w.dl, C, lane_prev_f(Z, 0.f));
    }
    __device__ __forceinline__ float decay_incoming2(float Lt, float Y0, const DecayW &w, float *Yend) {
        const float Z = wscan_decay(Lt, w);
        if (lane == 63) L->wf[sl][wv][0] = Z;
        __syncthreads();
        float C = Y0, Cin = Y0;
#pragma unroll
        for (int v = 0; v < 4; v++) { C = fmaf(C, w.d64, L->wf[sl][v][0]); Cin = (v + 1 == wv) ? C : Cin; }
        sl ^= 1;
        *Yend = C;
        return fmaf(w.dl, Cin, lane_prev_f(Z, 0.f));
    }
    __device__ __forceinline__ double excl_add_d(double tot, double *total, bool flag, bool *any_flag) {
        const double inc = wscan_add_d(tot);
        const bool wany = __any(flag) != 0;
        if (lane == 63) L->wd[sl][wv][0] = inc;
        if (lane == 0) L->wi[sl][wv][0] = wany ? 1 : 0;
        __syncthreads();
        double pre = 0.0, all = 0.0; int fl = 0;
#pragma unroll
        for (int v = 0; v < 4; v++) { const double t = L->wd[sl][v][0]; all += t; pre += (v < wv) ? t : 0.0; fl |= L->wi[sl][v][0]; }
        sl ^= 1;
        *total = all; *any_flag = fl != 0;
        return pre + (inc - tot);
    }
    __device__ __forceinline__ float excl_add_f(float tot, float *total) {
        const float inc = wscan_add_f(tot);
        if (lane == 63) L->wf[sl][wv][0] = inc;
        __syncthreads();
        float pre = 0.f, all = 0.f;
#pragma unroll
        for (int v = 0; v < 4; v++) { const float t = L->wf[sl][v][0]; all += t; pre += (v < wv) ? t : 0.f; }
        sl ^= 1;
        *total = all;
        return pre + lane_prev_f(inc, 0.f);
    }
    __device__ __forceinline__ void excl_add_max_i(int a, int m, int *pre_a, int *tot_a, int *pre_m, int *tot_m) {
        const int ia = wscan_add_i(a), im = wscan_max_i(m);
        if (lane == 63) { L->wi[sl][wv][0] = ia; L->wi[sl][wv][1] = im; }
        __syncthreads();
        int pa = 0, ta = 0, pm = -0x7fffffff - 1, tm = -0x7fffffff - 1;
#pragma unroll
        for (int v = 0; v < 4; v++) {
            const int xa = L->wi[sl][v][0], xm = L->wi[sl][v][1];
            ta += xa; tm = xm > tm ? xm : tm;
            if (v < wv) { pa += xa; pm = xm > pm ? xm : pm; }
        }
        sl ^= 1;
        const int ea = ia - a, em = lane_prev_i(im, -0x7fffffff - 1);
        *pre_a = pa + ea; *tot_a = ta; *pre_m = em > pm ? em : pm; *tot_m = tm;
    }
    __device__ __forceinline__ void reduce_max4(int &a, int &b, int &c, int &d) {
        a = wscan_max_i(a); b = wscan_max_i(b); c = wscan_max_i(c); d = wscan_max_i(d);
        if (lane == 63) { L->wi[sl][wv][0] = a; L->wi[sl][wv][1] = b; L->wi[sl][wv][2] = c; L->wi[sl][wv][3] = d; }
        __syncthreads();
        a = b = c = d = IMIN;
#pragma unroll
        for (int v = 0; v < 4; v++) {
            const int xa = L->wi[sl][v][0], xb = L->wi[sl][v][1], xc = L->wi[sl][v][2], xd = L->wi[sl][v][3];
            a = xa > a ? xa : a; b = xb > b ? xb : b; c = xc > c ? xc : c; d = xd > d ? xd : d;
        }
        sl ^= 1;
    }
    __device__ __forceinline__ float from_left2(float mine, float first, float *last) {
        L->edge[tid] = mine;
        __syncthreads();
        const float v = tid ? L->edge[tid - 1] : first;
        *last = L->edge[FB_T - 1];
        __syncthreads();
        return v;
    }
    __device__ __forceinline__ float from_left(float mine, float first) {
        L->edge[tid] = mine;
        __syncthreads();
        const float v = tid ? L->edge[tid - 1] : first;
        __syncthreads();
        return v;
    }
};

struct PssSt { float acc, mean, pdp; int lock_cnt, unlock_cnt; int minimized; };
__device__ __forceinline__ float pss_step(PssSt &s, float alpha, float la, float keep, bool locked, int tag, float err) {
    const bool rst = !locked;
    s.pdp = rst ? 0.f : s.pdp; s.acc = rst ? 0.f : s.acc; s.mean = rst ? 0.f : s.mean;
    s.minimized = s.minimized && !rst; s.lock_cnt = rst ? 0 : s.lock_cnt; s.unlock_cnt = rst ? 0 : s.unlock_cnt;
    const float used = s.pdp;
    const bool call = tag >= 0;
    const float error = s.minimized ? err : err * 10.0f;
    const float c4 = 0.785398185253143310546875f;
    const float nacc = fminf(fmaxf(s.acc + alpha * error, -c4), c4);
    const float nmean = la * error + s.mean * keep;
    const bool small = fabsf(nmean) < 0.001f;
    const int lc1 = s.lock_cnt + ((small && !s.minimized) ? 1 : 0);
    const int uc1 = s.unlock_cnt + ((!small && s.minimized) ? 1 : 0);
    const bool nmin = small ? (s.minimized || lc1 > 3 * SINCOS_N) : (s.minimized && !(uc1 > 3 * SINCOS_N));
    s.acc = call ? nacc : s.acc; s.mean = call ? nmean : s.mean; s.minimized = call ? nmin : s.minimized;
    s.lock_cnt = call ? (small ? lc1 : 0) : s.lock_cnt; s.unlock_cnt = call ? (small ? 0 : uc1) : s.unlock_cnt;
    s.pdp = call ? nacc : ((tag == -1) ? 0.f : s.pdp);
    return used;
}

__device__ __forceinline__ void meta_snapshot(ChanState *st, const ChanParams &P, float pdp, float mean, bool minimized, bool locked) {
    const bool lk = P.fm_mode != 2 && locked;
    st->meta_pss_deg = (float)((double)pdp / 3.14159265358979323846 * 180.0f);
    st->meta_pss_change = mean * 1000;
    st->meta_pss_state = (P.pss_active && lk) ? (minimized ? 2 : 1) : 0;
}

constexpr float AFC_EXACT_THR = 0.15f;
struct StageBArgs { DeviceTables T; DeviceBuffers B; CallGeom G; int C; };
typedef const StageBArgs __attribute__((address_space(4))) *StageBArgsP;
#define SB_ARGS_FRESH() asm volatile("" : "+s"(ka))

__device__ __forceinline__ bool all_in(const float *v, float limit) {
    unsigned m = __float_as_uint(v[0]);
#pragma unroll
    for (int i = 1; i < FB_K; i++) m = max(m, __float_as_uint(v[i]));
    return m < __float_as_uint(limit);
}

struct Aff { float A, Bv; };
template <int CTRL, int RM> __device__ __forceinline__ Aff aff_step(Aff c) {
    const float pA = dppf<CTRL, RM>(1.f, c.A);
    float pB;
    if constexpr (RM == 0xf) pB = dppzf<CTRL>(c.Bv); else pB = dppf<CTRL, RM>(0.f, c.Bv);
    Aff r; r.Bv = fmaf(c.A, pB, c.Bv); r.A = c.A * pA;
    return r;
}
__device__ __forceinline__ Aff wscan_aff(Aff v) {
    v = aff_step<0x111, 0xf>(v); v = aff_step<0x112, 0xf>(v); v = aff_step<0x114, 0xf>(v); v = aff_step<0x118, 0xf>(v);
    v = aff_step<0x142, 0xa>(v); v = aff_step<0x143, 0xc>(v);
    return v;
}

#ifndef SB_ABLATE
#define SB_ABLATE 0
#endif
#ifndef SB_SEED_ROUNDS
#define SB_SEED_ROUNDS 2
#endif
#ifndef SB_NEWTON_TOL
#define SB_NEWTON_TOL 2e-3f
#endif
constexpr float PLL_NEWTON_TOL = SB_NEWTON_TOL;
constexpr float PLL_GUARD = 0.12f;
constexpr int PLL_NEWTON_MAX = 10;

template <int PART>
__global__ __launch_bounds__(FB_T, PART == 0 ? SB_WG_PER_SIMD : 4) void stageb_kernel(StageBArgs by_value_never_touched) {
    StageBArgsP ka = (StageBArgsP)__builtin_amdgcn_kernarg_segment_ptr();
#define T (ka->T)
#define B (ka->B)
#define G (ka->G)
    const int C = ka->C;
    __shared__ ScanLds lds;
    __shared__ struct { float afc, x0, old, lock; int locked, stable; PssSt ps; float de_l, de_r; int calls; int newton_ok; } cy;
    constexpr int XF = 2 * fftc::LDS_N;
    __shared__ __attribute__((aligned(16))) float big[XF + 2 * FB_W];
    float2 *const X = reinterpret_cast<float2 *>(big);
    float *er = big;
    int *pk = reinterpret_cast<int *>(big) + FB_W;
    static_assert(2 * FB_W <= XF, "er and pk live in the convolution buffer");
    float *const park_dem = big + XF, *const park_cur = big + XF + FB_W;
    float *const sq_lo = big, *const sq_hi = big + FB_W, *const sq_b = big + 2 * FB_W, *const sq_wa = big + 3 * FB_W, *const sq_wb = big + 4 * FB_W;
    float *const pout = sq_lo;
    static_assert(5 * FB_W <= XF + 2 * FB_W && (FB_W % 4) == 0, "the rows fit the block");
    __shared__ __attribute__((aligned(16))) DecayTab<(PART == 0 ? 4 : 2)> dtab;
    const int ch = blockIdx.x + G.ch0;
    if (ch >= C) return;
#ifdef SB_POISON_LDS
    for (int i = threadIdx.x; i < XF + 2 * FB_W; i += FB_T) big[i] = __int_as_float(0x7fc0dead);
    for (int i = threadIdx.x; i < (int)(sizeof(lds) / 4); i += FB_T) reinterpret_cast<int *>(&lds)[i] = 0x7fc0dead;
    __syncthreads();
#endif
    WG wg; wg.L = &lds; wg.tid = threadIdx.x; wg.lane = threadIdx.x & 63; wg.wv = threadIdx.x >> 6; wg.sl = 0;
    const ChanParams &P = B.params[ch];
    ChanState *st = B.state + ch;
    const int nj = (int)(G.J1 - G.J0);
#ifdef SB_PHASE_CYCLES
    const bool dbg_on = (B.dbg != nullptr) && (threadIdx.x == 0);
    unsigned long long dbg_acc[9] = {0, 0, 0, 0, 0, 0, 0, 0, 0};
    unsigned long long dbg_t = dbg_on ? clock64() : 0ull;
#define SB_TICK1(k) SB_TICK(k)
#else
#define SB_TICK1(k) asm volatile("; SB_PHASE_END " #k " F%c0" :: "i"(SB_FASTFLAG))
#endif
#ifdef SB_FINE_TICKS
    __shared__ unsigned long long ft_acc[64];
    const bool ft_on = (B.dbg != nullptr) && (threadIdx.x == 0);
    if (threadIdx.x < 64) ft_acc[threadIdx.x] = 0ull;
    __syncthreads();
    unsigned long long ft_t = ft_on ? clock64() : 0ull;
#endif
    const bool stereo_possible = P.fm_mode != 2, auto_mono = P.auto_mono != 0, pss_active = P.pss_active != 0;
    const bool special = P.decoder <= 2 || P.squelch_mode != 0;
    const bool pss_on = stereo_possible && pss_active;
    const int my_count0 = st->my_count;
    const int jx = (SINCOS_N >> 1) - my_count0;
    const int zdelay = special ? 0 : T.front_sets[P.front_set].delay_fm;
    const float2 *const zr = B.zring + (size_t)ch * (G.ring_mask + 1);
    const int64_t callJ0 = G.J0;
    const int zmask = G.ring_mask;
    auto fetch = [&](int j0, int seg0, int w, float2 *z) {
        const int delay = zdelay;
        const int64_t base = callJ0 + seg0;
        if (w == FB_W && base - 2 - delay >= 0) {
            const int rmask = zmask;
            const int r0 = (int)((base - delay) & rmask) + j0 - 2;
            if (!__any(r0 < 0 || r0 + FB_K + 1 > rmask)) {
                const float2 *p = zr + r0;
#pragma unroll
                for (int t = 0; t < FB_K + 2; t++) z[t] = p[t];
                return;
            }
#pragma unroll
            for (int t = 0; t < FB_K + 2; t++) z[t] = zr[(r0 + t) & rmask];
            return;
        }
#pragma unroll
        for (int t = 0; t < FB_K + 2; t++) {
            const int jr = j0 - 2 + t;
            const int64_t jj = base + (jr < w ? jr : w - 1);
            const int64_t s = jj - delay;
            z[t] = jj < 0 ? make_float2(__builtin_nanf(""), 0.f) : (s >= 0 ? zr[s & zmask] : make_float2(0.f, 0.f));
        }
    };
    if (threadIdx.x == 0) {
        cy.afc = st->fm_afc; cy.x0 = st->pil_phase; cy.old = st->pil_old; cy.lock = st->pil_lock;
        cy.locked = st->pil_locked; cy.stable = st->pil_stable; cy.newton_ok = st->pll_newton_ok;
        PssSt ps;
        ps.acc = st->pss_acc; ps.mean = st->pss_mean; ps.pdp = st->pilot_delay_pss;
        ps.lock_cnt = st->pss_lock_cnt; ps.unlock_cnt = st->pss_unlock_cnt; ps.minimized = st->pss_minimized != 0;
        if (P.actions & (ACT_TRIGGER_FREQ | ACT_RESTART_PSS)) {
            ps.pdp = 0.f; ps.acc = 0.f; ps.minimized = false; ps.mean = 0.f; ps.lock_cnt = 0; ps.unlock_cnt = 0;
            if (P.actions & ACT_TRIGGER_FREQ) st->fade_start_frame = G.M0;
        }
        cy.ps = ps; cy.de_l = st->de_l; cy.de_r = st->de_r;
        cy.calls = 0;
    }
    const int64_t pss_count0 = st->pss_count;
    if (threadIdx.x < 64) {
        if (PART != 2) { store_decay(&dtab, DEC_AFC, T.afc_l2, threadIdx.x); store_decay(&dtab, DEC_LOCK, T.lock_l2, threadIdx.x); }
        if (PART != 1) { store_decay(&dtab, DEC_PSSMEAN, T.pssmean_l2, threadIdx.x); store_decay(&dtab, DEC_DEEMPH, P.deemph_l2, threadIdx.x); }
    }
    float2 zn[FB_K + 2];
    if (PART != 2 && !special) fetch((int)threadIdx.x * FB_K, 0, nj < FB_W ? nj : FB_W, zn);
    __syncthreads();
    bool newton_ok_next = st->pll_newton_ok != 0;
    bool afc_big_next = P.pll_seq == 0 && !special && fabsf(__int_as_float(__builtin_amdgcn_readfirstlane(__float_as_int(st->fm_afc)))) > AFC_EXACT_THR;
    auto segment = [&](auto fast_tag, auto exact_tag, const int seg0) {
        constexpr bool FAST = decltype(fast_tag)::value;
        constexpr bool EXACT = decltype(exact_tag)::value;
        constexpr int SB_FASTFLAG = FAST ? 1 : 0;
        const bool afc_big = EXACT && afc_big_next;
        int tid = threadIdx.x;
        asm volatile("" : "+v"(tid));
        wg.tid = tid; wg.lane = tid & 63; wg.wv = tid >> 6;
        const int lane = wg.lane;
        const int j0 = tid * FB_K;
        const int w = FAST ? FB_W : ((nj - seg0) < FB_W ? (nj - seg0) : FB_W);
        const bool lastseg = seg0 + FB_W >= nj;
        const int nv = FAST ? FB_K : w - j0;
        const bool owner = FAST ? (tid == FB_T - 1) : (nv >= 1 && nv <= FB_K);
        const int il = FAST ? FB_K - 1 : nv - 1;
        const int ix = FAST ? -1 : jx - seg0 - j0;

        SB_FT(0); SB_FTW(1);
        float dem[FB_K], cur[FB_K];
        bool locked[FB_K];
        bool all_locked;
        bool none_locked = false;
        uint8_t *const lockm = B.w_lockm + (size_t)ch * B.lockm_stride + (size_t)(seg0 / FB_W) * FB_T + tid;
        if constexpr (PART != 2) {
        if (!special) {
        float res[FB_K];
        if (SB_ABLATE & 1) {
#pragma unroll
            for (int i = 0; i < FB_K; i++) res[i] = zn[i + 2].x;
        } else {
            const int decoder = P.decoder;
            float2 lim[FB_K + 2];
#pragma unroll
            for (int t = 0; t < FB_K + 2; t++) lim[t] = (!FAST && zn[t].x != zn[t].x) ? make_float2((float)0.01, (float)0.01) : limiter_fast(zn[t]);
            bool exact_disc = false;
            if constexpr (EXACT) {
                exact_disc = P.pll_seq == 1 || afc_big;
                if (exact_disc) {
#pragma unroll
                    for (int t = 0; t < FB_K + 2; t++) lim[t] = (!FAST && zn[t].x != zn[t].x) ? make_float2((float)0.01, (float)0.01) : limiter(zn[t]);
                }
            }
            SB_FT(2);
            if (decoder == 5) {
                int index[FB_K];
#pragma unroll
                for (int i = 0; i < FB_K; i++) {
                    const float I = lim[i + 2].x, Q = lim[i + 2].y, I1 = lim[i + 1].x, Q1 = lim[i + 1].y;
                    const float r = (float)((double)(I1 * Q - Q1 * I + 1) / 2.0);
                    int ixx = (int)floorf(r * (float)ARCSINE_N);
                    ixx = ixx < 0 ? 0 : ixx;
                    index[i] = ixx >= ARCSINE_N ? ARCSINE_N : ixx;
                }
#pragma unroll
                for (int i = 0; i < FB_K; i++) res[i] = T.arcsine[index[i]];
            } else if (decoder == 6) {
#pragma unroll
                for (int i = 0; i < FB_K; i++) {
                    const float I = lim[i + 2].x, Q = lim[i + 2].y, I1 = lim[i + 1].x, Q1 = lim[i + 1].y;
                    const float Scaler = (float)1.4142135623730951;
                    const float r = (I1 * (Q - lim[i].y) - Q1 * (I - lim[i].x));
                    res[i] = exact_disc ? r / ((I1 * I1 + Q1 * Q1) * Scaler) : fdiv_fast(r, (I1 * I1 + Q1 * Q1) * Scaler);
                }
            } else {
                AtanArmF arm[FB_K];
                bool odd = false;
#pragma unroll
                for (int i = 0; i < FB_K; i++) {
                    const float I = lim[i + 2].x, Q = lim[i + 2].y, I1 = lim[i + 1].x, Q1 = lim[i + 1].y;
                    arm[i] = atan_arm_plain(Q * I1 - I * Q1, I * I1 + Q * Q1, &odd);
                }
                SB_FT(3);
                float tv[FB_K];
#pragma unroll
                for (int i = 0; i < FB_K; i++) tv[i] = T.atan_ppy[arm[i].idx];
                SB_FTW(4);
#pragma unroll
                for (int i = 0; i < FB_K; i++) res[i] = arm[i].A + (arm[i].neg ? -tv[i] : tv[i]);
                if (exact_disc) {
#pragma unroll
                    for (int i = 0; i < FB_K; i++) {
                        const float I = lim[i + 2].x, Q = lim[i + 2].y, I1 = lim[i + 1].x, Q1 = lim[i + 1].y;
                        res[i] = lut_atan2(T.atan_ppy, Q * I1 - I * Q1, I * I1 + Q * Q1);
                    }
                } else
                if (__any(odd)) {
#pragma unroll
                    for (int i = 0; i < FB_K; i++) {
                        const float I = lim[i + 2].x, Q = lim[i + 2].y, I1 = lim[i + 1].x, Q1 = lim[i + 1].y;
                        res[i] = lut_atan2_fast(T.atan_ppy, Q * I1 - I * Q1, I * I1 + Q * Q1);
                    }
                }
            }
#pragma unroll
            for (int i = 0; i < FB_K; i++) res[i] = (i < nv) ? res[i] : 0.f;
        }
        SB_FT(5);
        SB_ARGS_FRESH(); SB_TICK1(0);

        if (SB_ABLATE & 2) {
#pragma unroll
            for (int i = 0; i < FB_K; i++) dem[i] = res[i];
        } else {
            const float fmDcAlpha = 0.0001f, c1 = 1 - fmDcAlpha;
            float Lt = 0.f;
#pragma unroll
            for (int i = 0; i < FB_K; i++) Lt = c1 * Lt + fmDcAlpha * res[i];
            float afc_next;
            float afc = wg.decay_incoming2(Lt, cy.afc, load_decay(&dtab, DEC_AFC, lane), &afc_next);
            afc_big_next = P.pll_seq == 0 && fabsf(__int_as_float(__builtin_amdgcn_readfirstlane(__float_as_int(afc_next)))) > AFC_EXACT_THR;
            bool afc_exact = false;
            if constexpr (EXACT) {
                if (P.pll_seq == 1 || afc_big) {
                    const float afc0 = cy.afc;
                    for (int pass = 0; pass < 8; pass++) {
                        float o = afc;
#pragma unroll
                        for (int i = 0; i < FB_K; i++) if (i < nv) o = c1 * o + fmDcAlpha * res[i];
                        float po = dppf<0x138, 0xf>(0.f, o);
                        if (lane == 63) lds.wf[wg.sl][wg.wv][2] = o;
                        __syncthreads();
                        if (lane == 0) po = wg.wv ? lds.wf[wg.sl][(wg.wv + 3) & 3][2] : afc0;
                        wg.sl ^= 1;
                        const double d = (nv >= 1) ? (double)po - (double)afc : 0.0;
                        double total; bool any;
                        const double pre = wg.excl_add_d(d, &total, d != 0.0, &any);
                        if (!any) { afc_exact = true; break; }
                        afc = (float)((double)afc + (pre + d));
                    }
                }
            }
            float afc_end = 0.f;
            const float K_FM = T.K_FM, K_FM_rcp = T.K_FM_rcp;
#pragma unroll
            for (int i = 0; i < FB_K; i++) {
                afc = c1 * afc + fmDcAlpha * res[i];
                dem[i] = fdiv_const(20.0f * (res[i] - afc) * 1.0f, K_FM, K_FM_rcp);
                if (i == il) afc_end = afc;
                if (i == ix && i < nv) st->meta_dc_if = afc;
            }
            if (lastseg && owner) st->fm_afc = afc_end;
            if (afc_exact) { if (owner) cy.afc = afc_end; }
            else if (tid == 0) cy.afc = afc_next;
        }
        } else {
#pragma unroll
            for (int i = 0; i < FB_K; i++) dem[i] = (i < nv) ? B.w_osc[widx((int64_t)(seg0 + j0 + i), ch, G.pitch)] : 0.f;
        }
        SB_FT(6);
        SB_ARGS_FRESH(); SB_TICK1(1);

        float osc[FB_K];
        float osc_in;
        if (SB_ABLATE & 4) {
#pragma unroll
            for (int i = 0; i < FB_K; i++) { cur[i] = dem[i]; osc[i] = dem[i]; }
            osc_in = dem[0];
        } else {
            const float gain = T.pil_gain, omega = T.pil_omega;
            const double SC64 = T.sincos_C;
            const float P32 = 6.2831855f, C32 = T.wrap32_c, INV2PI32 = 0.159154943f;
            const bool wrap_ok = T.wrap32_ok != 0;
            float x0 = cy.x0;
            if (!(x0 >= 0.f && x0 < P32)) x0 = pi_constrain(x0);
            float g[FB_K];
#pragma unroll
            for (int i = 0; i < FB_K; i++) g[i] = (i < nv) ? (5 * dem[i]) * gain : 0.f;
            float ph[FB_K];
            float nxl = 0.f;
            const int pll_mode = P.pll_seq;
            bool exact_pending = EXACT;
            const bool guard_seg = pll_mode == 0 && EXACT;
            bool seq = false;
            bool failsafe = false;
            bool force_plain = false;
            auto eval = [&](int i, float phase, float *nx_out, float *val_out) {
                int idx = (int)((double)phase * SC64);
                idx = (int)min((unsigned)idx, (unsigned)idx - (unsigned)SINCOS_N);
                const float o = sin_idx_hw(idx);
                const float perr = (5 * dem[i]) * o;
                const float t = phase + perr * gain;
                const float val = t + omega;
                const float wrapped = wrap_ok ? (val - P32) + C32 : (float)((double)val - FMX_2PI);
                cur[i] = t; osc[i] = o;
                *val_out = val;
                *nx_out = (val < P32) ? val : wrapped;
            };
            auto into_range = [&](float phase) {
                const double pd = (double)phase;
                const float pw = (float)(pd - floor(pd * (1.0 / FMX_2PI)) * FMX_2PI);
                return (phase >= 0.f && phase < P32) ? phase : ((pw >= 0.f && pw < P32) ? pw : 0.f);
            };
            {
                float rv[FB_K];
                const double tb = ((double)x0 + (double)j0 * (double)omega) * (1.0 / FMX_2PI);
                const float tbf = (float)(tb - floor(tb));
#pragma unroll
                for (int i = 0; i < FB_K; i++) { const float v = tbf + (float)i * (omega * INV2PI32); rv[i] = v - floorf(v); }
                float cor[FB_K];
#pragma unroll
                for (int i = 0; i < FB_K; i++) cor[i] = 0.f;
#pragma unroll
                for (int round = 0; round < SB_SEED_ROUNDS; round++) {
                    float c[FB_K], run;
#pragma unroll
                    for (int i = 0; i < FB_K; i++) {
                        const float sv = g[i] * __builtin_amdgcn_sinf(round == 0 ? rv[i] : rv[i] + cor[i] * INV2PI32);
                        if (i == 0) { c[i] = 0.f; run = sv; } else { c[i] = run; run += sv; }
                    }
                    float total;
                    const float pre = wg.excl_add_f(run, &total);
#pragma unroll
                    for (int i = 0; i < FB_K; i++) cor[i] = pre + c[i];
                }
#pragma unroll
                for (int i = 0; i < FB_K; i++) {
                    float v = rv[i] + cor[i] * INV2PI32;
                    v = (v - floorf(v)) * P32;
                    ph[i] = (j0 + i == 0) ? x0 : (v < P32 ? v : 0.f);
                }
            }
            SB_FT(7);
            bool open_ = true;
            const double x0d = (double)x0;
            for (int it = 0; ; it++) {
                float ph_next = 0.f;
                if (seq) {
                    __syncthreads();
                    const bool plain = !EXACT || failsafe || force_plain || !wrap_ok;
                    bool cyc_ok = false;
                    if constexpr (EXACT) {
                    if (!plain) {
                        constexpr int CYC_LMAX = 12, CYC_MAXPASS = 10, CYC_RUNS = FB_T;
                        float *const cg = big + 2 * FB_W, *const cd = big + 3 * FB_W;
                        int *const canc = reinterpret_cast<int *>(big + 4 * FB_W), *const cK = canc + CYC_RUNS + 8;
#pragma unroll
                        for (int i = 0; i < FB_K; i++) if (i < nv) { cg[j0 + i] = ph[i]; cd[j0 + i] = 5 * dem[i]; }
                        __syncthreads();
                        bool af[FB_K]; int cnt = 0;
                        {
                            float prev = (j0 > 0 && nv > 0) ? cg[j0 - 1] : 0.f;
#pragma unroll
                            for (int i = 0; i < FB_K; i++) {
                                af[i] = i < nv && (j0 + i == 0 || (ph[i] >= 4.0f && prev < 4.0f));
                                cnt += af[i] ? 1 : 0; prev = ph[i];
                            }
                        }
                        int pre, nc, dm1, dm2;
                        wg.excl_add_max_i(cnt, 0, &pre, &nc, &dm1, &dm2);
#pragma unroll
                        for (int i = 0; i < FB_K; i++) if (af[i]) { if (pre < CYC_RUNS) canc[pre] = j0 + i; pre++; }
                        if (tid == 0) canc[nc < CYC_RUNS ? nc : CYC_RUNS] = w;
                        cK[tid] = 0;
                        __syncthreads();
                        const int c = tid;
                        const bool runner = c < nc && nc <= CYC_RUNS;
                        const int s_ = runner ? canc[c] : 0, len = runner ? canc[c + 1] - s_ : 0;
                        const bool has_next = runner && c + 1 < nc;
                        const float gs = runner ? cg[s_] : 4.0f, ge = has_next ? cg[s_ + len] : 4.0f;
                        bool fail = nc > CYC_RUNS || (runner && (len > CYC_LMAX || len < 1));
                        constexpr float Uq = 4.76837158203125e-07f;
                        int passes = 0;
                        for (; passes < CYC_MAXPASS; passes++) {
                            const int Kc = cK[c], Kn = (c + 1 < CYC_RUNS) ? cK[c + 1] : 0;
                            float x = (c == 0) ? x0 : gs + (float)Kc * Uq;
                            if (runner && c > 0 && !(x >= 4.0f && x < 8.0f)) fail = true;
                            for (int i = 0; i < CYC_LMAX; i++) {
                                if (runner && i < len) {
                                    pout[s_ + i] = x;
                                    int idx = (int)((double)x * SC64);
                                    idx = idx >= SINCOS_N ? idx - SINCOS_N : idx;
                                    const float val = (x + (cd[s_ + i] * sin_idx_hw(idx)) * gain) + omega;
                                    fail = fail || !(__float_as_uint(val) < __float_as_uint(2.f * P32));
                                    x = (val < P32) ? val : (val - P32) + C32;
                                }
                            }
                            int d = 0;
                            if (has_next && !fail) {
                                const float dq = (x - (ge + (float)Kn * Uq)) * 2097152.0f;
                                const float dr = rintf(dq);
                                if (!(dq == dr) || !(fabsf(dr) < 4096.f)) fail = true; else d = (int)dr;
                            }
                            int preD, totD, preM, totM;
                            wg.excl_add_max_i(d, (d != 0 ? 1 : 0) | (fail ? 2 : 0), &preD, &totD, &preM, &totM);
                            if (totM >= 2) break;
                            if (totM == 0) { cyc_ok = true; break; }
                            cK[c] = Kc + preD;
                            __syncthreads();
                        }
                        if (B.dbg && tid == 0) { B.dbg[(size_t)ch * DBG_SLOTS + 28] += passes + 1; B.dbg[(size_t)ch * DBG_SLOTS + 29] += 1; B.dbg[(size_t)ch * DBG_SLOTS + 30] += cyc_ok ? 0 : 1; }
                        __syncthreads();
                    }
                    }
                    const bool spec = EXACT && !plain && !cyc_ok;
                    if constexpr (EXACT) {
                    if (spec) {
                        constexpr double INVC = FMX_2PI / SINCOS_N;
#pragma unroll
                        for (int i = 0; i < FB_K; i++) {
                            float clo = 0.f, chi = 0.f, bb = 0.f, wa = 0.f, wb = 0.f;
                            if (i < nv) {
                                int idx = (int)((double)ph[i] * SC64);
                                idx = (int)min((unsigned)idx, (unsigned)idx - (unsigned)SINCOS_N);
                                idx = (unsigned)idx < (unsigned)SINCOS_N ? idx : 0;
                                const bool lower = (double)ph[i] < ((double)idx + 0.5) * INVC;
                                int klo = lower ? idx - 1 : idx;
                                klo = klo < 0 ? 0 : (klo > SINCOS_N - 2 ? SINCOS_N - 2 : klo);
                                const float d5 = 5 * dem[i];
                                clo = (d5 * sin_idx_hw(klo)) * gain; chi = (d5 * sin_idx_hw(klo + 1)) * gain;
                                const float bh = (float)((double)(klo + 1) * INVC);
                                bb = ((int)((double)bh * SC64) >= klo + 1) ? bh : __int_as_float(__float_as_int(bh) + 1);
                                const float vg = (ph[i] + (idx == klo ? clo : chi)) + omega;
                                const bool wr = !(vg < P32);
                                wa = wr ? -P32 : 0.f; wb = wr ? C32 : 0.f;
                            }
                            sq_lo[j0 + i] = clo; sq_hi[j0 + i] = chi; sq_b[j0 + i] = bb; sq_wa[j0 + i] = wa; sq_wb[j0 + i] = wb;
                        }
                    }
                    }
                    if (plain) {
#pragma unroll
                        for (int i = 0; i < FB_K; i++) if (i < nv) sq_hi[j0 + i] = dem[i];
                    }
                    SB_FT(33);
                    __syncthreads();
                    SB_FT(34);
                    if constexpr (EXACT)
                    if (tid == 0 && spec) {
                        float x = x0;
                        auto one = [&](float clo, float chi, float bb, float wa, float wb) {
                            const float xin = x;
                            const float xl = (((xin + clo) + omega) + wa) + wb, xh = (((xin + chi) + omega) + wa) + wb;
                            x = (xin < bb) ? xl : xh;
                            return xin;
                        };
                        const float4 *qlo = reinterpret_cast<const float4 *>(sq_lo), *qhi = reinterpret_cast<const float4 *>(sq_hi), *qb = reinterpret_cast<const float4 *>(sq_b),
                                     *qwa = reinterpret_cast<const float4 *>(sq_wa), *qwb = reinterpret_cast<const float4 *>(sq_wb);
                        float4 r0 = qlo[0], r1 = qhi[0], r2 = qb[0], r3 = qwa[0], r4 = qwb[0];
                        const int nq = (w + 3) >> 2;
                        for (int q = 0; q < nq; q++) {
                            const int qn = (q + 1 < FB_W / 4) ? q + 1 : q;
                            const float4 n0 = qlo[qn], n1 = qhi[qn], n2 = qb[qn], n3 = qwa[qn], n4 = qwb[qn];
                            float4 o;
                            o.x = one(r0.x, r1.x, r2.x, r3.x, r4.x); o.y = one(r0.y, r1.y, r2.y, r3.y, r4.y);
                            o.z = one(r0.z, r1.z, r2.z, r3.z, r4.z); o.w = one(r0.w, r1.w, r2.w, r3.w, r4.w);
                            reinterpret_cast<float4 *>(pout)[q] = o;
                            r0 = n0; r1 = n1; r2 = n2; r3 = n3; r4 = n4;
                        }
                    }
                    if (tid == 0 && plain) {
                        float phase = x0;
                        for (int j = 0; j < w; j++) {
                            const float d5 = 5 * sq_hi[j];
                            pout[j] = phase;
                            int idx = (int)((double)phase * SC64);
                            idx = idx >= SINCOS_N ? idx - SINCOS_N : idx;
                            const float val = (phase + (d5 * sin_idx_hw(idx)) * gain) + omega;
                            phase = (val >= 0.f && val < P32) ? val : pi_constrain(val);
                        }
                    }
                    if (tid == 0) {
                        if (failsafe) st->pll_replays += 1;
                        else if (guard_seg && !force_plain) st->pll_exact_segs += 1;
                        if (B.dbg && force_plain) B.dbg[(size_t)ch * DBG_SLOTS + 15] += 1;
                    }
                    SB_FT(35);
                    __syncthreads();
#pragma unroll
                    for (int i = 0; i < FB_K; i++) ph[i] = (i < nv) ? pout[j0 + i] : 0.f;
                    ph_next = (j0 + FB_K < w) ? pout[j0 + FB_K] : 0.f;
                    __syncthreads();
                    SB_FT(36);
                }
                float nx[FB_K], val[FB_K];
                if (__any(!all_in(ph, P32))) {
#pragma unroll
                    for (int i = 0; i < FB_K; i++) ph[i] = into_range(ph[i]);
                }
#pragma unroll
                for (int i = 0; i < FB_K; i++) eval(i, ph[i], &nx[i], &val[i]);
                if (__any(!all_in(val, 2.f * P32))) {
#pragma unroll
                    for (int i = 0; i < FB_K; i++) nx[i] = pi_constrain(val[i]);
                }
                SB_FT(8);
                if (seq || it > 0) {
                    int wopen = (!seq && __any(open_)) ? 1 : 0;
                    if (seq && !failsafe && !force_plain) {
                        bool defect = false;
#pragma unroll
                        for (int i = 0; i < FB_K; i++)
                            defect = defect || (j0 + i + 1 < w && __float_as_int(nx[i]) != __float_as_int(i + 1 < FB_K ? ph[i + 1 < FB_K ? i + 1 : i] : ph_next));
                        wopen |= __any(defect) ? 2 : 0;
                    }
                    if (lane == 63) lds.wf[wg.sl][wg.wv][1] = osc[FB_K - 1];
                    if (lane == 0) lds.wi[wg.sl][wg.wv][1] = wopen;
                    const float cold = cy.old;
                    __syncthreads();
                    const int anyopen = lds.wi[wg.sl][0][1] | lds.wi[wg.sl][1][1] | lds.wi[wg.sl][2][1] | lds.wi[wg.sl][3][1];
                    const float from_prev_wave = lds.wf[wg.sl][(wg.wv + 3) & 3][1], old_next = lds.wf[wg.sl][3][1];
                    wg.sl ^= 1;
                    if (anyopen & 2) { force_plain = true; continue; }
                    if (!anyopen) {
                        osc_in = dppf<0x138, 0xf>(0.f, osc[FB_K - 1]);
                        if (lane == 0) osc_in = wg.wv ? from_prev_wave : cold;
                        if (tid == 0) cy.old = old_next;
#pragma unroll
                        for (int i = 0; i < FB_K; i++) if (i == il) nxl = nx[i];
                        if (B.dbg && tid == 0 && !seq) { B.dbg[(size_t)ch * DBG_SLOTS + 8] += it; B.dbg[(size_t)ch * DBG_SLOTS + 11] += 1; }
                        break;
                    }
                }
                SB_FT(9);
                double e[FB_K], tot = 0.0;
#pragma unroll
                for (int i = 0; i < FB_K; i++) { e[i] = tot; tot += (i < nv) ? (double)nx[i] - (double)ph[i] : 0.0; }
                double pre;
                {
                    const double inc = wscan_add_d(tot);
                    if (lane == 63) lds.wd[wg.sl][wg.wv][0] = inc;
                    __syncthreads();
                    pre = inc - tot;
#pragma unroll
                    for (int v = 0; v < 3; v++) pre += (v < wg.wv) ? lds.wd[wg.sl][v][0] : 0.0;
                    wg.sl ^= 1;
                }
                if (it == PLL_NEWTON_MAX - 1) { seq = true; failsafe = true; continue; }
                float d[FB_K], c[FB_K];
#pragma unroll
                for (int i = 0; i < FB_K; i++) {
                    d[i] = (i < nv) ? (float)((x0d + (pre + e[i])) - (double)ph[i]) : 0.f;
                    c[i] = g[i] * __builtin_amdgcn_cosf(ph[i] * INV2PI32);
                }
                {
                    unsigned m = __float_as_uint(d[0]) & 0x7fffffffu;
#pragma unroll
                    for (int i = 1; i < FB_K; i++) m = max(m, __float_as_uint(d[i]) & 0x7fffffffu);
                    if (__any(!(m < __float_as_uint(3.0f)))) {
#pragma unroll
                        for (int i = 0; i < FB_K; i++) {
                            double dd = (x0d + (pre + e[i])) - (double)ph[i];
                            dd = dd > 3.14159265358979323846 ? dd - FMX_2PI : (dd < -3.14159265358979323846 ? dd + FMX_2PI : dd);
                            d[i] = (i < nv) ? (float)dd : 0.f;
                        }
                    }
                }
                Aff m; m.A = 1.f; m.Bv = 0.f;
#pragma unroll
                for (int i = 0; i < FB_K; i++) { m.Bv = fmaf(1.f + c[i], m.Bv, c[i] * d[i]); m.A *= 1.f + c[i]; }
                const Aff ain = wscan_aff(m);
                if (lane == 63) { lds.wf[wg.sl][wg.wv][2] = ain.A; lds.wf[wg.sl][wg.wv][3] = ain.Bv; }
                __syncthreads();
                float S = 0.f;
#pragma unroll
                for (int v = 0; v < 3; v++) if (v < wg.wv) S = fmaf(lds.wf[wg.sl][v][2], S, lds.wf[wg.sl][v][3]);
                wg.sl ^= 1;
                {
                    const float eA = dppf<0x138, 0xf>(1.f, ain.A), eB = dppf<0x138, 0xf>(0.f, ain.Bv);
                    S = fmaf(eA, S, eB);
                }
                float dmax = 0.f;
#pragma unroll
                for (int i = 0; i < FB_K; i++) {
                    if (i < nv) {
                        dmax = fmaxf(dmax, fabsf(d[i] + S));
                        ph[i] = (j0 + i == 0) ? x0 : (float)((x0d + (pre + e[i])) + (double)S);
                    }
                    S = fmaf(1.f + c[i], S, c[i] * d[i]);
                }
                SB_FT(10);
                open_ = !(dmax < PLL_NEWTON_TOL);
                if (exact_pending) { seq = true; exact_pending = false; }
            }
            SB_FT(11);
            if (owner) { const float xe = (nxl >= 0.f && nxl < P32) ? nxl : 0.f; cy.x0 = xe; if (lastseg) st->pil_phase = xe; }
            if (lastseg && owner) {
                float oe = 0.f;
#pragma unroll
                for (int i = 0; i < FB_K; i++) if (i == il) oe = osc[i];
                st->pil_old = oe;
            }
        }
        SB_FT(12);
        SB_ARGS_FRESH(); SB_TICK1(2);

        if (SB_ABLATE & 8) {
#pragma unroll
            for (int i = 0; i < FB_K; i++) locked[i] = osc[i] > 0.f;
            all_locked = osc_in > 0.f;
        } else {
            const float lockA = 1.0f / 3000.0f;
            const double keep = 1.0 - (double)lockA;
            const float keepf = (float)keep;
            const float omega = T.pil_omega, romega = T.pil_omega_rcp;
            float xq[FB_K];
            {
                float old = osc_in;
#pragma unroll
                for (int i = 0; i < FB_K; i++) {
                    const float quadRef = fdiv_const(osc[i] - old, omega, romega);
                    old = osc[i];
                    xq[i] = (i < nv) ? lockA * (-quadRef * (5 * dem[i])) : 0.f;
                }
            }
            float Lt = 0.f;
#pragma unroll
            for (int i = 0; i < FB_K; i++) Lt = xq[i] + Lt * keepf;
            SB_FT(13);
            float lock_next;
            const int locked0 = cy.locked, stable0 = cy.stable;
            float lock = wg.decay_incoming2(Lt, cy.lock, load_decay(&dtab, DEC_LOCK, lane), &lock_next);
            bool lock_exact = false;
            if constexpr (EXACT) {
                if (P.pll_seq == 1) {
                    const float lock0 = cy.lock;
                    for (int pass = 0; pass < 8; pass++) {
                        float o = lock;
#pragma unroll
                        for (int i = 0; i < FB_K; i++) if (i < nv) o = (float)((double)xq[i] + (double)o * keep);
                        float po = dppf<0x138, 0xf>(0.f, o);
                        if (lane == 63) lds.wf[wg.sl][wg.wv][2] = o;
                        __syncthreads();
                        if (lane == 0) po = wg.wv ? lds.wf[wg.sl][(wg.wv + 3) & 3][2] : lock0;
                        wg.sl ^= 1;
                        const double d = (nv >= 1) ? (double)po - (double)lock : 0.0;
                        double total; bool any;
                        const double pre = wg.excl_add_d(d, &total, d != 0.0, &any);
                        if (!any) { lock_exact = true; break; }
                        lock = (float)((double)lock + (pre + d));
                    }
                }
            }
            bool hi[FB_K]; int lastf = -1; float lock_end = 0.f, lock_x = 0.f;
            float lock_min = 1.0f;
#pragma unroll
            for (int i = 0; i < FB_K; i++) {
                lock = (float)((double)xq[i] + (double)lock * keep);
                hi[i] = lock > 0.07f;
                lock_min = (i < nv) ? fminf(lock_min, lock) : lock_min;
                if (i < nv && !hi[i]) lastf = j0 + i;
                if (i == il) lock_end = lock;
                if (i == ix) lock_x = lock;
            }
            SB_FT(14);
            int preF = -1, totF = -1;
            bool anynear;
            {
                const int wlow = (__any(lastf >= 0) ? 1 : 0) | (__any(!(lock_min > PLL_GUARD)) ? 2 : 0);
                if (lane == 0) lds.wi[wg.sl][wg.wv][2] = wlow;
                __syncthreads();
                const int anyw = lds.wi[wg.sl][0][2] | lds.wi[wg.sl][1][2] | lds.wi[wg.sl][2][2] | lds.wi[wg.sl][3][2];
                const int anylow = anyw & 1;
                anynear = (anyw & 2) != 0;
                wg.sl ^= 1;
                if (anylow) { int cnt_dummy, tot_dummy; wg.excl_add_max_i(0, lastf, &cnt_dummy, &tot_dummy, &preF, &totF); }
            }
            {
                int F = preF;
#pragma unroll
                for (int i = 0; i < FB_K; i++) {
                    if (i < nv && !hi[i]) F = j0 + i;
                    const bool lk = (F < 0) && (locked0 != 0 || stable0 + (j0 + i) + 1 > (SINCOS_N >> 1));
                    locked[i] = lk;
                    if (i == ix && i < nv) {
                        st->meta_locked = (stereo_possible && lk) ? 1 : 0;
                        st->meta_lock_strength = stereo_possible ? lock_x : 0.f;
                    }
                }
            }
            all_locked = totF < 0 && (locked0 != 0 || stable0 + 1 > (SINCOS_N >> 1));
            none_locked = locked0 == 0 && !(stable0 + w > (SINCOS_N >> 1));
            int nl, ns;
            if (totF < 0) { nl = (locked0 != 0 || stable0 + w > (SINCOS_N >> 1)) ? 1 : 0;
                            ns = locked0 ? stable0 : (stable0 + w < (SINCOS_N >> 1) + 1 ? stable0 + w : (SINCOS_N >> 1) + 1); }
            else { nl = 0; ns = w - 1 - totF; }
            const int nok = (nl && !anynear) ? 1 : 0;
            newton_ok_next = nok != 0;
            if (lastseg && owner) { st->pil_lock = lock_end; st->pil_locked = nl; st->pil_stable = ns; st->pll_newton_ok = nok; }
            if (tid == 0) { cy.locked = nl; cy.stable = ns; cy.newton_ok = nok; if (!lock_exact) cy.lock = lock_next; }
            if (lock_exact && owner) cy.lock = lock_end;
        }
        SB_FT(15);
        if (PART == 1 || B.rows_on) {
            const size_t lrow = (size_t)ch * B.lin_rows + seg0 + j0;
            float *wd = B.w_dem + lrow, *wc = B.w_cur + lrow;
#pragma unroll
            for (int i = 0; i < FB_K; i++) if (i < nv) { wd[i] = dem[i]; wc[i] = cur[i]; }
        }
        SB_FT(16);
        SB_ARGS_FRESH(); SB_TICK1(3);
        if constexpr (PART == 1) {
            unsigned m = (all_locked ? 0x80u : 0u) | (none_locked ? 0x40u : 0u);
#pragma unroll
            for (int i = 0; i < FB_K; i++) m |= locked[i] ? (1u << i) : 0u;
            *lockm = (uint8_t)m;
            if (!lastseg && !special) { const int wn = (nj - seg0 - FB_W) < FB_W ? (nj - seg0 - FB_W) : FB_W; fetch(j0, seg0 + FB_W, wn, zn); }
        }
        } else {
            const size_t lrow = (size_t)ch * B.lin_rows + seg0 + j0;
            const float *wd = B.w_dem + lrow, *wc = B.w_cur + lrow;
            const unsigned m = *lockm;
#pragma unroll
            for (int i = 0; i < FB_K; i++) { dem[i] = (i < nv) ? wd[i] : 0.f; cur[i] = (i < nv) ? wc[i] : 0.f; locked[i] = ((m >> i) & 1u) != 0; }
            all_locked = (m & 0x80u) != 0; none_locked = (m & 0x40u) != 0;
        }
        if constexpr (PART != 1) {

        const int calls_before = cy.calls;
        float2 *sring = B.sring + (size_t)ch * (G.sring_mask + 1);
        const int smask = G.sring_mask;
        if (pss_on && !(auto_mono && none_locked)) {
            const int64_t i0 = pss_count0 + calls_before;
            float2 a[8];
            const int64_t first = i0 - (PSS_DELAY + PSS_TAPS - 1);
            if (FAST && first >= 0) {
                const int r0 = (int)(first & smask) + tid;
#pragma unroll
                for (int p = 0; p < 7; p++) a[p] = sring[(r0 + FB_T * p) & smask];
                static_assert(FB_T * 7 < FB_W + PSS_TAPS - 1 && FB_W + PSS_TAPS - 1 <= FB_T * 8, "which window entries are padding");
                a[7] = (tid < FB_W + PSS_TAPS - 1 - FB_T * 7) ? sring[(r0 + FB_T * 7) & smask] : make_float2(0.f, 0.f);
            } else {
#pragma unroll
                for (int p = 0; p < 8; p++) {
                    const int n = tid + FB_T * p;
                    const int64_t idx = first + n;
                    a[p] = (n < w + PSS_TAPS - 1 && idx >= 0) ? sring[idx & smask] : make_float2(0.f, 0.f);
                }
            }
#pragma unroll
            for (int i = 0; i < FB_K; i += 2) {
                *reinterpret_cast<float2 *>(&park_dem[j0 + i]) = make_float2(dem[i], dem[i + 1]);
                *reinterpret_cast<float2 *>(&park_cur[j0 + i]) = make_float2(cur[i], cur[i + 1]);
            }
            SB_FT(17); SB_FTW(18);
            fftc::convolve(tid, a, X, T.fft_w, T.pss_hs);
            SB_FT(19);
            __syncthreads();
#pragma unroll
            for (int p = 0; p < 8; p++) {
                const int m = tid + FB_T * p - (PSS_TAPS - 1);
                if (m >= 0 && m < FB_W) er[m] = a[p].x * a[p].y;
            }
#pragma unroll
            for (int i = 0; i < FB_K; i += 2) {
                const float2 d2 = *reinterpret_cast<const float2 *>(&park_dem[j0 + i]), c2 = *reinterpret_cast<const float2 *>(&park_cur[j0 + i]);
                dem[i] = d2.x; dem[i + 1] = d2.y; cur[i] = c2.x; cur[i + 1] = c2.y;
            }
        }
        __syncthreads();
        SB_FT(20);
        SB_ARGS_FRESH(); SB_TICK1(4);

        int tag[FB_K];
        int ncalls;
        int firstU = -0x7fffffff - 1, firstZ = -0x7fffffff - 1;
        if (all_locked) {
#pragma unroll
            for (int i = 0; i < FB_K; i++) tag[i] = stereo_possible ? (pss_active ? ((i < nv) ? j0 + i : -2) : -1) : -2;
            ncalls = pss_on ? w : 0;
            if (stereo_possible && !pss_active) firstZ = 0;
        } else {
            int ncall_t = 0;
#pragma unroll
            for (int i = 0; i < FB_K; i++) {
                const bool branch = stereo_possible && (locked[i] || !auto_mono);
                tag[i] = branch ? (pss_active ? 0 : -1) : -2;
                ncall_t += (i < nv && branch && pss_active) ? 1 : 0;
            }
            int preC, dm1, dm2;
            wg.excl_add_max_i(ncall_t, 0, &preC, &ncalls, &dm1, &dm2);
            int c = preC;
#pragma unroll
            for (int i = 0; i < FB_K; i++) if (tag[i] == 0) { tag[i] = (i < nv) ? c : -2; c += (i < nv) ? 1 : 0; }
            int anyl = 0, alll = 0;
#pragma unroll
            for (int i = 0; i < FB_K; i++) if (i < nv) {
                if (!locked[i]) { const int v = -(j0 + i); firstU = v > firstU ? v : firstU; }
                if (tag[i] == -1) { const int v = -(j0 + i); firstZ = v > firstZ ? v : firstZ; }
            }
            wg.reduce_max4(firstU, firstZ, anyl, alll);
        }
        if (tid == 0) cy.calls = calls_before + ncalls;

        SB_FT(21);
        float used[FB_K];
        {
            const PssSt s = cy.ps;
            const float alpha = T.pss_alpha, la = T.pss_lock_alpha, keep = 1.0f - la;
            const float c4 = 0.785398185253143310546875f;
            float err[FB_K];
#pragma unroll
            for (int i = 0; i < FB_K; i++) err[i] = (pss_on && tag[i] >= 0) ? er[tag[i]] : 0.f;
            const bool steady = pss_on && all_locked && ((s.minimized ? s.unlock_cnt : s.lock_cnt) + w <= 3 * SINCOS_N);
            const bool nocall = ncalls == 0;
            PssSt e = s;
            if (steady) {
                const bool mz = s.minimized;
                float xa[FB_K], er10[FB_K];
#pragma unroll
                for (int i = 0; i < FB_K; i++) { er10[i] = mz ? err[i] : err[i] * 10.0f; xa[i] = alpha * er10[i]; }
                float a[FB_K];
                const double a0 = (double)s.acc;
                float aend;
                bool changed = false;
                {
                    double d1[FB_K], ex[FB_K], tot = 0.0;
#pragma unroll
                    for (int i = 0; i < FB_K; i++) {
                        const float na = fminf(fmaxf(s.acc + xa[i], -c4), c4);
                        d1[i] = (i < nv) ? (double)na - (double)s.acc : 0.0;
                        ex[i] = tot; tot += d1[i];
                    }
                    double total; bool any;
                    const double pre = wg.excl_add_d(tot, &total, false, &any);
#pragma unroll
                    for (int i = 0; i < FB_K; i++) {
                        const double exact = a0 + (pre + ex[i]);
                        a[i] = (float)exact;
                        const float na = fminf(fmaxf(a[i] + xa[i], -c4), c4);
                        changed = changed || (i < nv && ((double)a[i] != exact || (double)na - (double)a[i] != d1[i]));
                    }
                    aend = (float)(a0 + total);
                    changed = changed || (double)aend != a0 + total;
                }
                SB_FT(22);
                const DecayW dw = load_decay(&dtab, DEC_PSSMEAN, lane);
                float Lt = 0.f;
#pragma unroll
                for (int i = 0; i < FB_K; i++) Lt = ((i < nv) ? la * er10[i] : 0.f) + Lt * keep;
                float mean_next;
                float mean;
                {
                    const float Z = wscan_decay(Lt, dw);
                    const int wch = __any(changed) ? 1 : 0;
                    if (lane == 63) lds.wf[wg.sl][wg.wv][0] = Z;
                    if (lane == 0) lds.wi[wg.sl][wg.wv][0] = wch;
                    __syncthreads();
                    float Cc = s.mean, Cin = s.mean;
#pragma unroll
                    for (int v = 0; v < 4; v++) { Cc = fmaf(Cc, dw.d64, lds.wf[wg.sl][v][0]); Cin = (v + 1 == wg.wv) ? Cc : Cin; }
                    changed = (lds.wi[wg.sl][0][0] | lds.wi[wg.sl][1][0] | lds.wi[wg.sl][2][0] | lds.wi[wg.sl][3][0]) != 0;
                    wg.sl ^= 1;
                    mean_next = Cc;
                    mean = fmaf(dw.dl, Cin, lane_prev_f(Z, 0.f));
                }
                SB_FT(23);
                int rounds = 1;
                if (changed) {
                    for (int it = 0; ; it++) {
                        double d[FB_K], ex[FB_K], tot = 0.0;
#pragma unroll
                        for (int i = 0; i < FB_K; i++) {
                            const float na = fminf(fmaxf(a[i] + xa[i], -c4), c4);
                            d[i] = (i < nv) ? (double)na - (double)a[i] : 0.0;
                            ex[i] = tot; tot += d[i];
                        }
                        double total; bool any;
                        const double pre = wg.excl_add_d(tot, &total, false, &any);
                        bool ch2 = false;
#pragma unroll
                        for (int i = 0; i < FB_K; i++) {
                            const float na = (float)(a0 + (pre + ex[i]));
                            ch2 = ch2 || (i < nv && __float_as_int(na) != __float_as_int(a[i]));
                            a[i] = na;
                        }
                        aend = (float)(a0 + total);
                        if (lane == 0) lds.wi[wg.sl][wg.wv][0] = 0;
                        if (__any(ch2) && lane == 0) lds.wi[wg.sl][wg.wv][0] = 1;
                        __syncthreads();
                        const int anych = lds.wi[wg.sl][0][0] | lds.wi[wg.sl][1][0] | lds.wi[wg.sl][2][0] | lds.wi[wg.sl][3][0];
                        wg.sl ^= 1;
                        rounds++;
                        if (!anych || it == PSS_MAX_ROUNDS - 1) break;
                    }
                }
                SB_FT(24);
                if (B.dbg && tid == 0) { B.dbg[(size_t)ch * DBG_SLOTS + 9] += rounds; B.dbg[(size_t)ch * DBG_SLOTS + 12] += 1; }
#pragma unroll
                for (int i = 0; i < FB_K; i++) used[i] = (j0 + i == 0) ? s.pdp : a[i];
                int lastS = -1, lastN = -1, d3 = 0, d4 = 0; float mean_end = 0.f;
#pragma unroll
                for (int i = 0; i < FB_K; i++) {
                    mean = la * er10[i] + mean * keep;
                    if (i < nv) { if (fabsf(mean) < 0.001f) lastS = j0 + i; else lastN = j0 + i; }
                    if (i == il) mean_end = mean;
                    if (i == ix && i < nv) meta_snapshot(st, P, fminf(fmaxf(a[i] + xa[i], -c4), c4), mean, mz, true);
                }
                SB_FT(25);
                wg.reduce_max4(lastS, lastN, d3, d4);
                if (tid == 0) {
                    const int lc0 = cy.ps.lock_cnt, uc0 = cy.ps.unlock_cnt;
                    const bool all_small = lastN < 0, any_small = lastS >= 0;
                    int lc, uc;
                    if (mz) { lc = all_small ? lc0 : 0; uc = any_small ? (w - 1 - lastS) : uc0 + w; }
                    else { lc = all_small ? lc0 + w : (w - 1 - lastN); uc = any_small ? 0 : uc0; }
                    cy.ps.acc = aend; cy.ps.pdp = aend; cy.ps.minimized = mz ? 1 : 0; cy.ps.lock_cnt = lc; cy.ps.unlock_cnt = uc;
                }
                if (owner) cy.ps.mean = mean_end;
            } else if (nocall) {
                const int fu = (firstU == -0x7fffffff - 1) ? 0x7fffffff : -firstU, fz = (firstZ == -0x7fffffff - 1) ? 0x7fffffff : -firstZ;
#pragma unroll
                for (int i = 0; i < FB_K; i++) used[i] = (j0 + i >= fu || j0 + i > fz) ? 0.f : s.pdp;
#pragma unroll
                for (int i = 0; i < FB_K; i++) if (i == ix && i < nv) {
                    const bool cleared = j0 + i >= fu;
                    meta_snapshot(st, P, (cleared || j0 + i >= fz) ? 0.f : s.pdp, cleared ? 0.f : s.mean, cleared ? false : s.minimized, locked[i]);
                }
                if (fu != 0x7fffffff) { e.pdp = 0.f; e.acc = 0.f; e.mean = 0.f; e.minimized = false; e.lock_cnt = 0; e.unlock_cnt = 0; }
                else if (fz != 0x7fffffff) e.pdp = 0.f;
                __syncthreads();
                if (tid == 0) cy.ps = e;
            } else {
                __syncthreads();
#pragma unroll
                for (int i = 0; i < FB_K; i++) if (i < nv) { pk[j0 + i] = ((tag[i] + 2) << 1) | (locked[i] ? 1 : 0); er[j0 + i] = err[i]; }
                __syncthreads();
                if (B.dbg && tid == 0) B.dbg[(size_t)ch * DBG_SLOTS + 10] += 1;
                if (tid == 0) {
                    PssSt r = s;
                    const int jxs = jx - seg0;
                    for (int j = 0; j < w; j++) {
                        const int p = pk[j];
                        er[j] = pss_step(r, alpha, la, keep, (p & 1) != 0, (p >> 1) - 2, er[j]);
                        if (j == jxs) meta_snapshot(st, P, r.pdp, r.mean, r.minimized, (p & 1) != 0);
                    }
                    cy.ps = r;
                }
                __syncthreads();
#pragma unroll
                for (int i = 0; i < FB_K; i++) used[i] = (i < nv) ? er[j0 + i] : 0.f;
            }
        }
        SB_FT(26);
        SB_ARGS_FRESH(); SB_TICK1(5);

        float2 x[FB_K];
        {
            constexpr double INV2PI = 1.0 / FMX_2PI;
            const int ssel = P.sound_sel; const float pano = (P.fm_mode == 1) ? P.panorama : 1.0f;
            const int icl = (int)((pss_count0 + calls_before) & smask);
            const float P32 = 6.2831855f, C32 = T.wrap32_c;
            const bool wrap_ok = T.wrap32_ok != 0;
            float sumv[FB_K], diffv[FB_K];
            const bool wide = __any(!all_in(cur, P32 + 0.5f)) || !wrap_ok;
#pragma unroll
            for (int i = 0; i < FB_K; i++) {
                float cc = (cur[i] < P32) ? cur[i] : (cur[i] - P32) + C32;
                if (wide) cc = pi_constrain(cur[i]);
                const float p = (float)(2 * ((double)cc + FMX_PI_4) - (double)used[i]);
                const double u = __builtin_amdgcn_fract((double)p * INV2PI);
                const int idx = (int)(u * (double)SINCOS_N);
                float2 e;
                sincos_idx_hw_bits(idx, &e.y, &e.x);
                float dif = 0.f;
                if (tag[i] != -2) {
                    if (tag[i] >= 0 && i < nv) sring[(icl + tag[i]) & smask] = make_float2(e.x * dem[i], e.y * dem[i]);
                    const float lut = (ssel == 6) ? e.y : e.x;
                    dif = 2.0f * (lut * dem[i]);
                }
                sumv[i] = dem[i]; diffv[i] = dif;
            }
            SB_FT(27);
            if (B.w_diff) {
                float *wf = B.w_diff + (size_t)ch * B.lin_rows + seg0 + j0;
#pragma unroll
                for (int i = 0; i < FB_K; i++) if (i < nv) wf[i] = diffv[i];
            }
#pragma unroll
            for (int i = 0; i < FB_K; i++) {
                const float sumLR = sumv[i];
                const float dw = diffv[i] * pano;
                const float left = sumLR + dw, right = sumLR - dw;
                float2 o;
                switch (ssel) {
                default:
                case 0: o = make_float2(left, right); break;
                case 1: o = make_float2(right, left); break;
                case 2: o = make_float2(left, left); break;
                case 3: o = make_float2(right, right); break;
                case 4: o = make_float2(sumLR, sumLR); break;
                case 5: case 6: o = make_float2(dw, dw); break;
                }
                x[i] = (i < nv) ? o : make_float2(0.f, 0.f);
            }
        }
        SB_FT(28);
        SB_ARGS_FRESH(); SB_TICK1(6);

        if (PART == 0 && !lastseg && !special) { const int wn = (nj - seg0 - FB_W) < FB_W ? (nj - seg0 - FB_W) : FB_W; fetch(j0, seg0 + FB_W, wn, zn); }
        SB_FT(29);
        if (G.no_deemph) {
            const int dmask = G.dring_mask;
            float2 *dr = B.dring + (size_t)ch * (dmask + 1);
            const int jb = (int)((G.J0 + seg0 + j0) & dmask);
#pragma unroll
            for (int i = 0; i < FB_K; i++) if (i < nv) dr[(jb + i) & dmask] = x[i];
        } else
        {
            const float a = P.deemph_alpha;
            const DecayW dw = load_decay(&dtab, DEC_DEEMPH, lane);
            float Ll = 0.f, Lr = 0.f;
#pragma unroll
            for (int i = 0; i < FB_K; i++) { Ll = (x[i].x - Ll) * a + Ll; Lr = (x[i].y - Lr) * a + Lr; }
            SB_FT(30);
            float yl, yr;
            {
                const float Zl = wscan_decay(Ll, dw), Zr = wscan_decay(Lr, dw);
                if (lane == 63) { lds.wf[wg.sl][wg.wv][0] = Zl; lds.wf[wg.sl][wg.wv][1] = Zr; }
                const float cl0 = cy.de_l, cr0 = cy.de_r;
                __syncthreads();
                float Cl = cl0, Cr = cr0;
                for (int v = 0; v < wg.wv; v++) { Cl = fmaf(Cl, dw.d64, lds.wf[wg.sl][v][0]); Cr = fmaf(Cr, dw.d64, lds.wf[wg.sl][v][1]); }
                wg.sl ^= 1;
                yl = fmaf(dw.dl, Cl, lane_prev_f(Zl, 0.f)); yr = fmaf(dw.dl, Cr, lane_prev_f(Zr, 0.f));
            }
            SB_FT(31);
            const int dmask = G.dring_mask;
            float2 *dr = B.dring + (size_t)ch * (dmask + 1);
            const int jb = (int)((G.J0 + seg0 + j0) & dmask);
            float el = 0.f, er_ = 0.f;
#pragma unroll
            for (int i = 0; i < FB_K; i++) {
                yl = (x[i].x - yl) * a + yl;
                yr = (x[i].y - yr) * a + yr;
                if (i < nv) dr[(jb + i) & dmask] = make_float2(yl, yr);
                if (i == il) { el = yl; er_ = yr; }
            }
            if (owner) { cy.de_l = el; cy.de_r = er_; }
        }
        SB_FT(32);
        SB_ARGS_FRESH(); SB_TICK1(7);
        }
    };
    for (int seg0 = 0; seg0 < nj; seg0 += FB_W) {
        const bool fast = (nj - seg0 >= FB_W) && !((unsigned)(jx - seg0) < (unsigned)FB_W) && (callJ0 + seg0 >= 2);
        const bool exact = PART != 2 && (P.pll_seq == 1 || (P.pll_seq == 0 && stereo_possible && !newton_ok_next) || afc_big_next);
        if (fast) { if (exact) segment(std::true_type{}, std::true_type{}, seg0); else segment(std::true_type{}, std::false_type{}, seg0); }
        else { if (exact) segment(std::false_type{}, std::true_type{}, seg0); else segment(std::false_type{}, std::false_type{}, seg0); }
    }
    __syncthreads();
    if (PART != 1 && threadIdx.x == 0) {
        const PssSt ps = cy.ps;
        st->pss_acc = ps.acc; st->pss_mean = ps.mean; st->pilot_delay_pss = ps.pdp;
        st->pss_lock_cnt = ps.lock_cnt; st->pss_unlock_cnt = ps.unlock_cnt; st->pss_minimized = ps.minimized ? 1 : 0;
        if (!G.no_deemph) { st->de_l = cy.de_l; st->de_r = cy.de_r; }
        int cnt = my_count0 + nj;
        if (cnt > (SINCOS_N >> 1)) {
            const float dcabs = (float)sqrt((double)st->dc_re * (double)st->dc_re + (double)st->dc_im * (double)st->dc_im);
            st->meta_dc_rf = P.dc_remove ? 20 * log10f(dcabs + 1.0f / 32768) : (float)-99.99;
            cnt -= (SINCOS_N >> 1) + 1;
        }
        st->my_count = cnt;
        st->pss_count = pss_count0 + cy.calls;
        st->pss_call_total = 0;
    }
    constexpr int SB_FASTFLAG = 2;
    SB_TICK1(8);
#ifdef SB_PHASE_CYCLES
    if (dbg_on) for (int k = 0; k < 9; k++) B.dbg[(size_t)ch * DBG_SLOTS + 16 + k] += dbg_acc[k];
#endif
#ifdef SB_FINE_TICKS
    __syncthreads();
    if (ft_on) for (int k = 0; k < 64; k++) B.dbg[(size_t)ch * DBG_SLOTS + 32 + k] += ft_acc[k];
#endif
    if (B.dbg && threadIdx.x == 0) {
        B.dbg[(size_t)ch * DBG_SLOTS + 13] = __float_as_uint(cy.x0); B.dbg[(size_t)ch * DBG_SLOTS + 14] = __float_as_uint(cy.lock);
    }
}
#undef T
#undef B
#undef G

void launch_demod_fused(const DeviceTables &T, const DeviceBuffers &B, const CallGeom &G, int C, hipStream_t s, const PrepassStreams *ps) {
    if (G.J1 - G.J0 <= 0) return;
    if (B.w_iq) launch_demod_prepass(T, B, G, C, s, ps);
    StageBArgs A; A.T = T; A.B = B; A.G = G; A.C = C;
    const bool split = stageb_two_kernels(C, G.n_cus, B.rows_on != 0, G.stageb_form, SB_WG_PER_SIMD);
    const unsigned grid = (unsigned)(G.ch_count > 0 ? G.ch_count : C);
    if (split) {
        hipLaunchKernelGGL(stageb_kernel<1>, dim3(grid), dim3(FB_T), 0, s, A); FMX_LAUNCHED();
        hipLaunchKernelGGL(stageb_kernel<2>, dim3(grid), dim3(FB_T), 0, s, A); FMX_LAUNCHED();
    } else {
        hipLaunchKernelGGL(stageb_kernel<0>, dim3(grid), dim3(FB_T), 0, s, A); FMX_LAUNCHED();
    }
}

}
```

Measured before the change: 278,200 MS/s.

## Add half-width fast segment form and snapshot-aware fast path in stage B

Stage B segments that hold the metadata snapshot index or are half-width tails were previously forced onto the general (bounds-checked) path. This adds a HALF_FAST template form where only the first two wavefronts do work, and lets full fast segments carry the snapshot through a compile-time-selected loop variant. It also caches loop-invariant channel params in shared memory and reads them via readfirstlane to keep them scalar. The cost is more template instantiations and code size, plus guarded zero-init in the half form. An env switch can disable it.

After: 275,600 MS/s. Within noise of the previous version (-0.9%).

```diff
diff --git a/sdr-j-fm_amd/csrc/fmx_api.hip b/sdr-j-fm_amd/csrc/fmx_api.hip
--- a/sdr-j-fm_amd/csrc/fmx_api.hip
+++ b/sdr-j-fm_amd/csrc/fmx_api.hip
@@ -15,9 +15,10 @@
 struct EnvSwitches {
     bool pieces_serial;
     bool tail_split;
+    bool stageb_tail_fast;
 };
 const EnvSwitches &env_switches() {
-    static const EnvSwitches sw{env_int("FMX_CALL_PIECES_SERIAL", 0) != 0, env_int("FMX_TAIL_SPLIT", 1) != 0};
+    static const EnvSwitches sw{env_int("FMX_CALL_PIECES_SERIAL", 0) != 0, env_int("FMX_TAIL_SPLIT", 1) != 0, env_int("FMX_STAGEB_TAIL_FAST", 1) != 0};
     return sw;
 }
 
@@ -976,6 +977,7 @@
     if (!h->call_scan.empty() && G.J1 > G.J0 && (rc = stage_scan(h, G, sa))) return rc;
     if (prof) HIPCHK(hipEventRecord(pr.e[1], sa));
     G.stageb_form = h->stageb_form.load(); G.no_deemph = h->ola_mode ? 1 : 0;
+    G.stageb_tail_fast = env_switches().stageb_tail_fast ? 1 : 0;
     const bool plain = plain_batch(PieceFlags{piped, h->ola_mode, h->B.w_iq != nullptr, h->cv_nt != 0, h->needs.rows_on, rds_running, h->gain_pending, G.stageb_form,
                                               G.J1 > G.J0, G.M1 > G.M0});
     const int second = env_switches().tail_split && plain ? second_group_channels(h->channels, h->n_cus) : 0;
diff --git a/sdr-j-fm_amd/csrc/fmx_internal.h b/sdr-j-fm_amd/csrc/fmx_internal.h
--- a/sdr-j-fm_amd/csrc/fmx_internal.h
+++ b/sdr-j-fm_amd/csrc/fmx_internal.h
@@ -195,6 +195,7 @@
     int32_t ch_count;
     int32_t ch0;
     int32_t host_count1;
+    int32_t stageb_tail_fast;
     int32_t parts, part_tiles;
 };
 struct FrontSnap { int32_t lo_phase, hist_fmt; float dc_re, dc_im; };
diff --git a/sdr-j-fm_amd/csrc/fmx_plan.h b/sdr-j-fm_amd/csrc/fmx_plan.h
--- a/sdr-j-fm_amd/csrc/fmx_plan.h
+++ b/sdr-j-fm_amd/csrc/fmx_plan.h
@@ -1,6 +1,12 @@
 #pragma once
 #include <cstdint>
 #include <vector>
+
+#ifdef __HIPCC__
+#define FMX_PLAN_HD __host__ __device__ __forceinline__
+#else
+#define FMX_PLAN_HD inline
+#endif
 
 namespace fmx {
 
@@ -92,6 +98,18 @@
     return rows_on && halves < whole;
 }
 
+enum class SegForm { FULL_FAST, HALF_FAST, GENERAL };
+struct SegChoice { SegForm form; bool snapshot; };
+FMX_PLAN_HD SegChoice stageb_segment_form(int nj, int seg0, int jx, int64_t callJ0, bool tail_fast) {
+    const int w = (nj - seg0) < STAGEB_SEG ? (nj - seg0) : STAGEB_SEG;
+    const bool snapshot = jx >= seg0 && jx - seg0 < w;
+    const bool behind_start = callJ0 + seg0 >= 2;
+    SegForm form = SegForm::GENERAL;
+    if (behind_start && w == STAGEB_SEG && (tail_fast || !snapshot)) form = SegForm::FULL_FAST;
+    else if (behind_start && w == STAGEB_SEG / 2 && tail_fast) form = SegForm::HALF_FAST;
+    return {form, snapshot};
+}
+
 inline int second_group_channels(int channels, int n_cus) {
     const int slots = STAGEB_WG_PER_CU * (n_cus > 0 ? n_cus : 256);
     if (channels <= slots) return 0;
diff --git a/sdr-j-fm_amd/csrc/fmx_stageb.hip b/sdr-j-fm_amd/csrc/fmx_stageb.hip
--- a/sdr-j-fm_amd/csrc/fmx_stageb.hip
+++ b/sdr-j-fm_amd/csrc/fmx_stageb.hip
@@ -209,11 +209,11 @@
     return used;
 }
 
-__device__ __forceinline__ void meta_snapshot(ChanState *st, const ChanParams &P, float pdp, float mean, bool minimized, bool locked) {
-    const bool lk = P.fm_mode != 2 && locked;
+__device__ __forceinline__ void meta_snapshot(ChanState *st, bool stereo_possible, bool pss_active, float pdp, float mean, bool minimized, bool locked) {
+    const bool lk = stereo_possible && locked;
     st->meta_pss_deg = (float)((double)pdp / 3.14159265358979323846 * 180.0f);
     st->meta_pss_change = mean * 1000;
-    st->meta_pss_state = (P.pss_active && lk) ? (minimized ? 2 : 1) : 0;
+    st->meta_pss_state = (pss_active && lk) ? (minimized ? 2 : 1) : 0;
 }
 
 constexpr float AFC_EXACT_THR = 0.15f;
@@ -304,12 +304,15 @@
     const bool stereo_possible = P.fm_mode != 2, auto_mono = P.auto_mono != 0, pss_active = P.pss_active != 0;
     const bool special = P.decoder <= 2 || P.squelch_mode != 0;
     const bool pss_on = stereo_possible && pss_active;
-    const int my_count0 = st->my_count;
+    const int my_count0 = __builtin_amdgcn_readfirstlane(st->my_count);
     const int jx = (SINCOS_N >> 1) - my_count0;
     const int zdelay = special ? 0 : T.front_sets[P.front_set].delay_fm;
     const float2 *const zr = B.zring + (size_t)ch * (G.ring_mask + 1);
     const int64_t callJ0 = G.J0;
     const int zmask = G.ring_mask;
+    const bool tail_fast = G.stageb_tail_fast != 0;
+    __shared__ struct { int decoder, pll_seq, sound_sel; float deemph_alpha, pano; } inv;
+    auto inv_i = [](const int &v) { return __builtin_amdgcn_readfirstlane(v); };
     auto fetch = [&](int j0, int seg0, int w, float2 *z) {
         const int delay = zdelay;
         const int64_t base = callJ0 + seg0;
@@ -346,6 +349,8 @@
         }
         cy.ps = ps; cy.de_l = st->de_l; cy.de_r = st->de_r;
         cy.calls = 0;
+        inv.decoder = P.decoder; inv.pll_seq = P.pll_seq; inv.sound_sel = P.sound_sel;
+        inv.deemph_alpha = P.deemph_alpha; inv.pano = (P.fm_mode == 1) ? P.panorama : 1.0f;
     }
     const int64_t pss_count0 = st->pss_count;
     if (threadIdx.x < 64) {
@@ -357,26 +362,40 @@
     __syncthreads();
     bool newton_ok_next = st->pll_newton_ok != 0;
     bool afc_big_next = P.pll_seq == 0 && !special && fabsf(__int_as_float(__builtin_amdgcn_readfirstlane(__float_as_int(st->fm_afc)))) > AFC_EXACT_THR;
-    auto segment = [&](auto fast_tag, auto exact_tag, const int seg0) {
-        constexpr bool FAST = decltype(fast_tag)::value;
+    auto segment = [&](auto form_tag, auto exact_tag, const int seg0, const bool snap) {
+        constexpr int NW = decltype(form_tag)::value;
+        constexpr bool FAST = NW != 0, HALF = NW == 2;
+        constexpr int SEGW = FAST ? NW * 64 * FB_K : FB_W;
         constexpr bool EXACT = decltype(exact_tag)::value;
-        constexpr int SB_FASTFLAG = FAST ? 1 : 0;
+        constexpr int SB_FASTFLAG = HALF ? 3 : (FAST ? 1 : 0);
         const bool afc_big = EXACT && afc_big_next;
         int tid = threadIdx.x;
         asm volatile("" : "+v"(tid));
         wg.tid = tid; wg.lane = tid & 63; wg.wv = tid >> 6;
         const int lane = wg.lane;
         const int j0 = tid * FB_K;
-        const int w = FAST ? FB_W : ((nj - seg0) < FB_W ? (nj - seg0) : FB_W);
+        const int w = FAST ? SEGW : ((nj - seg0) < FB_W ? (nj - seg0) : FB_W);
         const bool lastseg = seg0 + FB_W >= nj;
-        const int nv = FAST ? FB_K : w - j0;
-        const bool owner = FAST ? (tid == FB_T - 1) : (nv >= 1 && nv <= FB_K);
+        const bool active = !HALF || __builtin_amdgcn_readfirstlane(tid >> 6) < NW;
+        const int nv = FAST ? (active ? FB_K : 0) : w - j0;
+        const int nv_seg = nv;
+#define SB_IF_ACTIVE if (const int nv = FAST ? FB_K : nv_seg; (void)nv, active)
+        const bool owner = FAST ? (tid == SEGW / FB_K - 1) : (nv >= 1 && nv <= FB_K);
         const int il = FAST ? FB_K - 1 : nv - 1;
-        const int ix = FAST ? -1 : jx - seg0 - j0;
+        const int ix = jx - seg0 - j0;
+
+        auto snap_loop = [&](auto body) {
+            if constexpr (FAST) { if (snap) body(std::true_type{}); else body(std::false_type{}); } else body(std::true_type{});
+        };
+#define SNAP_HERE(sx) (decltype(sx)::value && i == ix && i < nv)
 
         SB_FT(0); SB_FTW(1);
         float dem[FB_K], cur[FB_K];
         bool locked[FB_K];
+        if constexpr (HALF) {
+#pragma unroll
+            for (int i = 0; i < FB_K; i++) { dem[i] = 0.f; cur[i] = 0.f; locked[i] = false; }
+        }
         bool all_locked;
         bool none_locked = false;
         uint8_t *const lockm = B.w_lockm + (size_t)ch * B.lockm_stride + (size_t)(seg0 / FB_W) * FB_T + tid;
@@ -386,14 +405,14 @@
         if (SB_ABLATE & 1) {
 #pragma unroll
             for (int i = 0; i < FB_K; i++) res[i] = zn[i + 2].x;
-        } else {
-            const int decoder = P.decoder;
+        } else SB_IF_ACTIVE {
+            const int decoder = inv_i(inv.decoder);
             float2 lim[FB_K + 2];
 #pragma unroll
             for (int t = 0; t < FB_K + 2; t++) lim[t] = (!FAST && zn[t].x != zn[t].x) ? make_float2((float)0.01, (float)0.01) : limiter_fast(zn[t]);
             bool exact_disc = false;
             if constexpr (EXACT) {
-                exact_disc = P.pll_seq == 1 || afc_big;
+                exact_disc = inv_i(inv.pll_seq) == 1 || afc_big;
                 if (exact_disc) {
 #pragma unroll
                     for (int t = 0; t < FB_K + 2; t++) lim[t] = (!FAST && zn[t].x != zn[t].x) ? make_float2((float)0.01, (float)0.01) : limiter(zn[t]);
@@ -452,6 +471,9 @@
             }
 #pragma unroll
             for (int i = 0; i < FB_K; i++) res[i] = (i < nv) ? res[i] : 0.f;
+        } else {
+#pragma unroll
+            for (int i = 0; i < FB_K; i++) res[i] = 0.f;
         }
         SB_FT(5);
         SB_ARGS_FRESH(); SB_TICK1(0);
@@ -462,14 +484,16 @@
         } else {
             const float fmDcAlpha = 0.0001f, c1 = 1 - fmDcAlpha;
             float Lt = 0.f;
-#pragma unroll
-            for (int i = 0; i < FB_K; i++) Lt = c1 * Lt + fmDcAlpha * res[i];
+            SB_IF_ACTIVE {
+#pragma unroll
+                for (int i = 0; i < FB_K; i++) Lt = c1 * Lt + fmDcAlpha * res[i];
+            }
             float afc_next;
             float afc = wg.decay_incoming2(Lt, cy.afc, load_decay(&dtab, DEC_AFC, lane), &afc_next);
-            afc_big_next = P.pll_seq == 0 && fabsf(__int_as_float(__builtin_amdgcn_readfirstlane(__float_as_int(afc_next)))) > AFC_EXACT_THR;
+            afc_big_next = inv_i(inv.pll_seq) == 0 && fabsf(__int_as_float(__builtin_amdgcn_readfirstlane(__float_as_int(afc_next)))) > AFC_EXACT_THR;
             bool afc_exact = false;
             if constexpr (EXACT) {
-                if (P.pll_seq == 1 || afc_big) {
+                if (inv_i(inv.pll_seq) == 1 || afc_big) {
                     const float afc0 = cy.afc;
                     for (int pass = 0; pass < 8; pass++) {
                         float o = afc;
@@ -490,13 +514,15 @@
             }
             float afc_end = 0.f;
             const float K_FM = T.K_FM, K_FM_rcp = T.K_FM_rcp;
-#pragma unroll
-            for (int i = 0; i < FB_K; i++) {
-                afc = c1 * afc + fmDcAlpha * res[i];
-                dem[i] = fdiv_const(20.0f * (res[i] - afc) * 1.0f, K_FM, K_FM_rcp);
-                if (i == il) afc_end = afc;
-                if (i == ix && i < nv) st->meta_dc_if = afc;
-            }
+            SB_IF_ACTIVE snap_loop([&](auto sx) {
+#pragma unroll
+                for (int i = 0; i < FB_K; i++) {
+                    afc = c1 * afc + fmDcAlpha * res[i];
+                    dem[i] = fdiv_const(20.0f * (res[i] - afc) * 1.0f, K_FM, K_FM_rcp);
+                    if (i == il) afc_end = afc;
+                    if (SNAP_HERE(sx)) st->meta_dc_if = afc;
+                }
+            });
             if (lastseg && owner) st->fm_afc = afc_end;
             if (afc_exact) { if (owner) cy.afc = afc_end; }
             else if (tid == 0) cy.afc = afc_next;
@@ -525,8 +551,12 @@
 #pragma unroll
             for (int i = 0; i < FB_K; i++) g[i] = (i < nv) ? (5 * dem[i]) * gain : 0.f;
             float ph[FB_K];
+            if constexpr (HALF) {
+#pragma unroll
+                for (int i = 0; i < FB_K; i++) { ph[i] = 0.f; osc[i] = 0.f; }
+            }
             float nxl = 0.f;
-            const int pll_mode = P.pll_seq;
+            const int pll_mode = inv_i(inv.pll_seq);
             bool exact_pending = EXACT;
             const bool guard_seg = pll_mode == 0 && EXACT;
             bool seq = false;
@@ -551,31 +581,39 @@
             };
             {
                 float rv[FB_K];
-                const double tb = ((double)x0 + (double)j0 * (double)omega) * (1.0 / FMX_2PI);
-                const float tbf = (float)(tb - floor(tb));
-#pragma unroll
-                for (int i = 0; i < FB_K; i++) { const float v = tbf + (float)i * (omega * INV2PI32); rv[i] = v - floorf(v); }
                 float cor[FB_K];
 #pragma unroll
-                for (int i = 0; i < FB_K; i++) cor[i] = 0.f;
+                for (int i = 0; i < FB_K; i++) { rv[i] = 0.f; cor[i] = 0.f; }
+                SB_IF_ACTIVE {
+                    const double tb = ((double)x0 + (double)j0 * (double)omega) * (1.0 / FMX_2PI);
+                    const float tbf = (float)(tb - floor(tb));
+#pragma unroll
+                    for (int i = 0; i < FB_K; i++) { const float v = tbf + (float)i * (omega * INV2PI32); rv[i] = v - floorf(v); }
+                }
 #pragma unroll
                 for (int round = 0; round < SB_SEED_ROUNDS; round++) {
-                    float c[FB_K], run;
-#pragma unroll
-                    for (int i = 0; i < FB_K; i++) {
-                        const float sv = g[i] * __builtin_amdgcn_sinf(round == 0 ? rv[i] : rv[i] + cor[i] * INV2PI32);
-                        if (i == 0) { c[i] = 0.f; run = sv; } else { c[i] = run; run += sv; }
+                    float c[FB_K], run = 0.f;
+#pragma unroll
+                    for (int i = 0; i < FB_K; i++) c[i] = 0.f;
+                    SB_IF_ACTIVE {
+#pragma unroll
+                        for (int i = 0; i < FB_K; i++) {
+                            const float sv = g[i] * __builtin_amdgcn_sinf(round == 0 ? rv[i] : rv[i] + cor[i] * INV2PI32);
+                            if (i == 0) { c[i] = 0.f; run = sv; } else { c[i] = run; run += sv; }
+                        }
                     }
                     float total;
                     const float pre = wg.excl_add_f(run, &total);
 #pragma unroll
                     for (int i = 0; i < FB_K; i++) cor[i] = pre + c[i];
                 }
-#pragma unroll
-                for (int i = 0; i < FB_K; i++) {
-                    float v = rv[i] + cor[i] * INV2PI32;
-                    v = (v - floorf(v)) * P32;
-                    ph[i] = (j0 + i == 0) ? x0 : (v < P32 ? v : 0.f);
+                SB_IF_ACTIVE {
+#pragma unroll
+                    for (int i = 0; i < FB_K; i++) {
+                        float v = rv[i] + cor[i] * INV2PI32;
+                        v = (v - floorf(v)) * P32;
+                        ph[i] = (j0 + i == 0) ? x0 : (v < P32 ? v : 0.f);
+                    }
                 }
             }
             SB_FT(7);
@@ -731,15 +769,21 @@
                     SB_FT(36);
                 }
                 float nx[FB_K], val[FB_K];
-                if (__any(!all_in(ph, P32))) {
-#pragma unroll
-                    for (int i = 0; i < FB_K; i++) ph[i] = into_range(ph[i]);
-                }
-#pragma unroll
-                for (int i = 0; i < FB_K; i++) eval(i, ph[i], &nx[i], &val[i]);
-                if (__any(!all_in(val, 2.f * P32))) {
-#pragma unroll
-                    for (int i = 0; i < FB_K; i++) nx[i] = pi_constrain(val[i]);
+                if constexpr (HALF) {
+#pragma unroll
+                    for (int i = 0; i < FB_K; i++) { nx[i] = 0.f; val[i] = 0.f; }
+                }
+                SB_IF_ACTIVE {
+                    if (__any(!all_in(ph, P32))) {
+#pragma unroll
+                        for (int i = 0; i < FB_K; i++) ph[i] = into_range(ph[i]);
+                    }
+#pragma unroll
+                    for (int i = 0; i < FB_K; i++) eval(i, ph[i], &nx[i], &val[i]);
+                    if (__any(!all_in(val, 2.f * P32))) {
+#pragma unroll
+                        for (int i = 0; i < FB_K; i++) nx[i] = pi_constrain(val[i]);
+                    }
                 }
                 SB_FT(8);
                 if (seq || it > 0) {
@@ -771,8 +815,14 @@
                 }
                 SB_FT(9);
                 double e[FB_K], tot = 0.0;
-#pragma unroll
-                for (int i = 0; i < FB_K; i++) { e[i] = tot; tot += (i < nv) ? (double)nx[i] - (double)ph[i] : 0.0; }
+                if constexpr (HALF) {
+#pragma unroll
+                    for (int i = 0; i < FB_K; i++) e[i] = 0.0;
+                }
+                SB_IF_ACTIVE {
+#pragma unroll
+                    for (int i = 0; i < FB_K; i++) { e[i] = tot; tot += (i < nv) ? (double)nx[i] - (double)ph[i] : 0.0; }
+                }
                 double pre;
                 {
                     const double inc = wscan_add_d(tot);
@@ -785,6 +835,12 @@
                 }
                 if (it == PLL_NEWTON_MAX - 1) { seq = true; failsafe = true; continue; }
                 float d[FB_K], c[FB_K];
+                Aff m; m.A = 1.f; m.Bv = 0.f;
+                if constexpr (HALF) {
+#pragma unroll
+                    for (int i = 0; i < FB_K; i++) { d[i] = 0.f; c[i] = 0.f; }
+                }
+                SB_IF_ACTIVE {
 #pragma unroll
                 for (int i = 0; i < FB_K; i++) {
                     d[i] = (i < nv) ? (float)((x0d + (pre + e[i])) - (double)ph[i]) : 0.f;
@@ -803,9 +859,9 @@
                         }
                     }
                 }
-                Aff m; m.A = 1.f; m.Bv = 0.f;
 #pragma unroll
                 for (int i = 0; i < FB_K; i++) { m.Bv = fmaf(1.f + c[i], m.Bv, c[i] * d[i]); m.A *= 1.f + c[i]; }
+                }
                 const Aff ain = wscan_aff(m);
                 if (lane == 63) { lds.wf[wg.sl][wg.wv][2] = ain.A; lds.wf[wg.sl][wg.wv][3] = ain.Bv; }
                 __syncthreads();
@@ -818,13 +874,15 @@
                     S = fmaf(eA, S, eB);
                 }
                 float dmax = 0.f;
-#pragma unroll
-                for (int i = 0; i < FB_K; i++) {
-                    if (i < nv) {
-                        dmax = fmaxf(dmax, fabsf(d[i] + S));
-                        ph[i] = (j0 + i == 0) ? x0 : (float)((x0d + (pre + e[i])) + (double)S);
-                    }
-                    S = fmaf(1.f + c[i], S, c[i] * d[i]);
+                SB_IF_ACTIVE {
+#pragma unroll
+                    for (int i = 0; i < FB_K; i++) {
+                        if (i < nv) {
+                            dmax = fmaxf(dmax, fabsf(d[i] + S));
+                            ph[i] = (j0 + i == 0) ? x0 : (float)((x0d + (pre + e[i])) + (double)S);
+                        }
+                        S = fmaf(1.f + c[i], S, c[i] * d[i]);
+                    }
                 }
                 SB_FT(10);
                 open_ = !(dmax < PLL_NEWTON_TOL);
@@ -852,7 +910,12 @@
             const float keepf = (float)keep;
             const float omega = T.pil_omega, romega = T.pil_omega_rcp;
             float xq[FB_K];
-            {
+            float Lt = 0.f;
+            if constexpr (HALF) {
+#pragma unroll
+                for (int i = 0; i < FB_K; i++) xq[i] = 0.f;
+            }
+            SB_IF_ACTIVE {
                 float old = osc_in;
 #pragma unroll
                 for (int i = 0; i < FB_K; i++) {
@@ -860,17 +923,16 @@
                     old = osc[i];
                     xq[i] = (i < nv) ? lockA * (-quadRef * (5 * dem[i])) : 0.f;
                 }
-            }
-            float Lt = 0.f;
-#pragma unroll
-            for (int i = 0; i < FB_K; i++) Lt = xq[i] + Lt * keepf;
+#pragma unroll
+                for (int i = 0; i < FB_K; i++) Lt = xq[i] + Lt * keepf;
+            }
             SB_FT(13);
             float lock_next;
             const int locked0 = cy.locked, stable0 = cy.stable;
             float lock = wg.decay_incoming2(Lt, cy.lock, load_decay(&dtab, DEC_LOCK, lane), &lock_next);
             bool lock_exact = false;
             if constexpr (EXACT) {
-                if (P.pll_seq == 1) {
+                if (inv_i(inv.pll_seq) == 1) {
                     const float lock0 = cy.lock;
                     for (int pass = 0; pass < 8; pass++) {
                         float o = lock;
@@ -891,15 +953,21 @@
             }
             bool hi[FB_K]; int lastf = -1; float lock_end = 0.f, lock_x = 0.f;
             float lock_min = 1.0f;
-#pragma unroll
-            for (int i = 0; i < FB_K; i++) {
-                lock = (float)((double)xq[i] + (double)lock * keep);
-                hi[i] = lock > 0.07f;
-                lock_min = (i < nv) ? fminf(lock_min, lock) : lock_min;
-                if (i < nv && !hi[i]) lastf = j0 + i;
-                if (i == il) lock_end = lock;
-                if (i == ix) lock_x = lock;
-            }
+            if constexpr (HALF) {
+#pragma unroll
+                for (int i = 0; i < FB_K; i++) hi[i] = true;
+            }
+            SB_IF_ACTIVE snap_loop([&](auto sx) {
+#pragma unroll
+                for (int i = 0; i < FB_K; i++) {
+                    lock = (float)((double)xq[i] + (double)lock * keep);
+                    hi[i] = lock > 0.07f;
+                    lock_min = (i < nv) ? fminf(lock_min, lock) : lock_min;
+                    if (i < nv && !hi[i]) lastf = j0 + i;
+                    if (i == il) lock_end = lock;
+                    if (decltype(sx)::value && i == ix) lock_x = lock;
+                }
+            });
             SB_FT(14);
             int preF = -1, totF = -1;
             bool anynear;
@@ -913,19 +981,19 @@
                 wg.sl ^= 1;
                 if (anylow) { int cnt_dummy, tot_dummy; wg.excl_add_max_i(0, lastf, &cnt_dummy, &tot_dummy, &preF, &totF); }
             }
-            {
+            SB_IF_ACTIVE snap_loop([&](auto sx) {
                 int F = preF;
 #pragma unroll
                 for (int i = 0; i < FB_K; i++) {
                     if (i < nv && !hi[i]) F = j0 + i;
                     const bool lk = (F < 0) && (locked0 != 0 || stable0 + (j0 + i) + 1 > (SINCOS_N >> 1));
                     locked[i] = lk;
-                    if (i == ix && i < nv) {
+                    if (SNAP_HERE(sx)) {
                         st->meta_locked = (stereo_possible && lk) ? 1 : 0;
                         st->meta_lock_strength = stereo_possible ? lock_x : 0.f;
                     }
                 }
-            }
+            });
             all_locked = totF < 0 && (locked0 != 0 || stable0 + 1 > (SINCOS_N >> 1));
             none_locked = locked0 == 0 && !(stable0 + w > (SINCOS_N >> 1));
             int nl, ns;
@@ -942,8 +1010,10 @@
         if (PART == 1 || B.rows_on) {
             const size_t lrow = (size_t)ch * B.lin_rows + seg0 + j0;
             float *wd = B.w_dem + lrow, *wc = B.w_cur + lrow;
-#pragma unroll
-            for (int i = 0; i < FB_K; i++) if (i < nv) { wd[i] = dem[i]; wc[i] = cur[i]; }
+            SB_IF_ACTIVE {
+#pragma unroll
+                for (int i = 0; i < FB_K; i++) if (i < nv) { wd[i] = dem[i]; wc[i] = cur[i]; }
+            }
         }
         SB_FT(16);
         SB_ARGS_FRESH(); SB_TICK1(3);
@@ -958,8 +1028,12 @@
             const size_t lrow = (size_t)ch * B.lin_rows + seg0 + j0;
             const float *wd = B.w_dem + lrow, *wc = B.w_cur + lrow;
             const unsigned m = *lockm;
-#pragma unroll
-            for (int i = 0; i < FB_K; i++) { dem[i] = (i < nv) ? wd[i] : 0.f; cur[i] = (i < nv) ? wc[i] : 0.f; locked[i] = ((m >> i) & 1u) != 0; }
+            SB_IF_ACTIVE {
+#pragma unroll
+                for (int i = 0; i < FB_K; i++) { dem[i] = (i < nv) ? wd[i] : 0.f; cur[i] = (i < nv) ? wc[i] : 0.f; }
+            }
+#pragma unroll
+            for (int i = 0; i < FB_K; i++) locked[i] = ((m >> i) & 1u) != 0;
             all_locked = (m & 0x80u) != 0; none_locked = (m & 0x40u) != 0;
         }
         if constexpr (PART != 1) {
@@ -973,10 +1047,13 @@
             const int64_t first = i0 - (PSS_DELAY + PSS_TAPS - 1);
             if (FAST && first >= 0) {
                 const int r0 = (int)(first & smask) + tid;
-#pragma unroll
-                for (int p = 0; p < 7; p++) a[p] = sring[(r0 + FB_T * p) & smask];
-                static_assert(FB_T * 7 < FB_W + PSS_TAPS - 1 && FB_W + PSS_TAPS - 1 <= FB_T * 8, "which window entries are padding");
-                a[7] = (tid < FB_W + PSS_TAPS - 1 - FB_T * 7) ? sring[(r0 + FB_T * 7) & smask] : make_float2(0.f, 0.f);
+                constexpr int NEED = SEGW + PSS_TAPS - 1;
+#pragma unroll
+                for (int p = 0; p < 8; p++) {
+                    if (FB_T * (p + 1) <= NEED) a[p] = sring[(r0 + FB_T * p) & smask];
+                    else if (FB_T * p >= NEED) a[p] = make_float2(0.f, 0.f);
+                    else a[p] = (tid < NEED - FB_T * p) ? sring[(r0 + FB_T * p) & smask] : make_float2(0.f, 0.f);
+                }
             } else {
 #pragma unroll
                 for (int p = 0; p < 8; p++) {
@@ -985,10 +1062,12 @@
                     a[p] = (n < w + PSS_TAPS - 1 && idx >= 0) ? sring[idx & smask] : make_float2(0.f, 0.f);
                 }
             }
-#pragma unroll
-            for (int i = 0; i < FB_K; i += 2) {
-                *reinterpret_cast<float2 *>(&park_dem[j0 + i]) = make_float2(dem[i], dem[i + 1]);
-                *reinterpret_cast<float2 *>(&park_cur[j0 + i]) = make_float2(cur[i], cur[i + 1]);
+            SB_IF_ACTIVE {
+#pragma unroll
+                for (int i = 0; i < FB_K; i += 2) {
+                    *reinterpret_cast<float2 *>(&park_dem[j0 + i]) = make_float2(dem[i], dem[i + 1]);
+                    *reinterpret_cast<float2 *>(&park_cur[j0 + i]) = make_float2(cur[i], cur[i + 1]);
+                }
             }
             SB_FT(17); SB_FTW(18);
             fftc::convolve(tid, a, X, T.fft_w, T.pss_hs);
@@ -999,10 +1078,12 @@
                 const int m = tid + FB_T * p - (PSS_TAPS - 1);
                 if (m >= 0 && m < FB_W) er[m] = a[p].x * a[p].y;
             }
-#pragma unroll
-            for (int i = 0; i < FB_K; i += 2) {
-                const float2 d2 = *reinterpret_cast<const float2 *>(&park_dem[j0 + i]), c2 = *reinterpret_cast<const float2 *>(&park_cur[j0 + i]);
-                dem[i] = d2.x; dem[i + 1] = d2.y; cur[i] = c2.x; cur[i + 1] = c2.y;
+            SB_IF_ACTIVE {
+#pragma unroll
+                for (int i = 0; i < FB_K; i += 2) {
+                    const float2 d2 = *reinterpret_cast<const float2 *>(&park_dem[j0 + i]), c2 = *reinterpret_cast<const float2 *>(&park_cur[j0 + i]);
+                    dem[i] = d2.x; dem[i + 1] = d2.y; cur[i] = c2.x; cur[i + 1] = c2.y;
+                }
             }
         }
         __syncthreads();
@@ -1063,20 +1144,28 @@
                 bool changed = false;
                 {
                     double d1[FB_K], ex[FB_K], tot = 0.0;
-#pragma unroll
-                    for (int i = 0; i < FB_K; i++) {
-                        const float na = fminf(fmaxf(s.acc + xa[i], -c4), c4);
-                        d1[i] = (i < nv) ? (double)na - (double)s.acc : 0.0;
-                        ex[i] = tot; tot += d1[i];
+                    if constexpr (HALF) {
+#pragma unroll
+                        for (int i = 0; i < FB_K; i++) { d1[i] = 0.0; ex[i] = 0.0; a[i] = 0.f; }
+                    }
+                    SB_IF_ACTIVE {
+#pragma unroll
+                        for (int i = 0; i < FB_K; i++) {
+                            const float na = fminf(fmaxf(s.acc + xa[i], -c4), c4);
+                            d1[i] = (i < nv) ? (double)na - (double)s.acc : 0.0;
+                            ex[i] = tot; tot += d1[i];
+                        }
                     }
                     double total; bool any;
                     const double pre = wg.excl_add_d(tot, &total, false, &any);
-#pragma unroll
-                    for (int i = 0; i < FB_K; i++) {
-                        const double exact = a0 + (pre + ex[i]);
-                        a[i] = (float)exact;
-                        const float na = fminf(fmaxf(a[i] + xa[i], -c4), c4);
-                        changed = changed || (i < nv && ((double)a[i] != exact || (double)na - (double)a[i] != d1[i]));
+                    SB_IF_ACTIVE {
+#pragma unroll
+                        for (int i = 0; i < FB_K; i++) {
+                            const double exact = a0 + (pre + ex[i]);
+                            a[i] = (float)exact;
+                            const float na = fminf(fmaxf(a[i] + xa[i], -c4), c4);
+                            changed = changed || (i < nv && ((double)a[i] != exact || (double)na - (double)a[i] != d1[i]));
+                        }
                     }
                     aend = (float)(a0 + total);
                     changed = changed || (double)aend != a0 + total;
@@ -1084,8 +1173,10 @@
                 SB_FT(22);
                 const DecayW dw = load_decay(&dtab, DEC_PSSMEAN, lane);
                 float Lt = 0.f;
-#pragma unroll
-                for (int i = 0; i < FB_K; i++) Lt = ((i < nv) ? la * er10[i] : 0.f) + Lt * keep;
+                SB_IF_ACTIVE {
+#pragma unroll
+                    for (int i = 0; i < FB_K; i++) Lt = ((i < nv) ? la * er10[i] : 0.f) + Lt * keep;
+                }
                 float mean_next;
                 float mean;
                 {
@@ -1137,13 +1228,15 @@
 #pragma unroll
                 for (int i = 0; i < FB_K; i++) used[i] = (j0 + i == 0) ? s.pdp : a[i];
                 int lastS = -1, lastN = -1, d3 = 0, d4 = 0; float mean_end = 0.f;
+                SB_IF_ACTIVE snap_loop([&](auto sx) {
 #pragma unroll
                 for (int i = 0; i < FB_K; i++) {
                     mean = la * er10[i] + mean * keep;
                     if (i < nv) { if (fabsf(mean) < 0.001f) lastS = j0 + i; else lastN = j0 + i; }
                     if (i == il) mean_end = mean;
-                    if (i == ix && i < nv) meta_snapshot(st, P, fminf(fmaxf(a[i] + xa[i], -c4), c4), mean, mz, true);
-                }
+                    if (SNAP_HERE(sx)) meta_snapshot(st, stereo_possible, pss_active, fminf(fmaxf(a[i] + xa[i], -c4), c4), mean, mz, true);
+                }
+                });
                 SB_FT(25);
                 wg.reduce_max4(lastS, lastN, d3, d4);
                 if (tid == 0) {
@@ -1159,10 +1252,11 @@
                 const int fu = (firstU == -0x7fffffff - 1) ? 0x7fffffff : -firstU, fz = (firstZ == -0x7fffffff - 1) ? 0x7fffffff : -firstZ;
 #pragma unroll
                 for (int i = 0; i < FB_K; i++) used[i] = (j0 + i >= fu || j0 + i > fz) ? 0.f : s.pdp;
+                if (!FAST || snap)
 #pragma unroll
                 for (int i = 0; i < FB_K; i++) if (i == ix && i < nv) {
                     const bool cleared = j0 + i >= fu;
-                    meta_snapshot(st, P, (cleared || j0 + i >= fz) ? 0.f : s.pdp, cleared ? 0.f : s.mean, cleared ? false : s.minimized, locked[i]);
+                    meta_snapshot(st, stereo_possible, pss_active, (cleared || j0 + i >= fz) ? 0.f : s.pdp, cleared ? 0.f : s.mean, cleared ? false : s.minimized, locked[i]);
                 }
                 if (fu != 0x7fffffff) { e.pdp = 0.f; e.acc = 0.f; e.mean = 0.f; e.minimized = false; e.lock_cnt = 0; e.unlock_cnt = 0; }
                 else if (fz != 0x7fffffff) e.pdp = 0.f;
@@ -1180,7 +1274,7 @@
                     for (int j = 0; j < w; j++) {
                         const int p = pk[j];
                         er[j] = pss_step(r, alpha, la, keep, (p & 1) != 0, (p >> 1) - 2, er[j]);
-                        if (j == jxs) meta_snapshot(st, P, r.pdp, r.mean, r.minimized, (p & 1) != 0);
+                        if (j == jxs) meta_snapshot(st, stereo_possible, pss_active, r.pdp, r.mean, r.minimized, (p & 1) != 0);
                     }
                     cy.ps = r;
                 }
@@ -1193,9 +1287,13 @@
         SB_ARGS_FRESH(); SB_TICK1(5);
 
         float2 x[FB_K];
-        {
+        if constexpr (HALF) {
+#pragma unroll
+            for (int i = 0; i < FB_K; i++) x[i] = make_float2(0.f, 0.f);
+        }
+        SB_IF_ACTIVE {
             constexpr double INV2PI = 1.0 / FMX_2PI;
-            const int ssel = P.sound_sel; const float pano = (P.fm_mode == 1) ? P.panorama : 1.0f;
+            const int ssel = inv_i(inv.sound_sel); const float pano = inv.pano;
             const int icl = (int)((pss_count0 + calls_before) & smask);
             const float P32 = 6.2831855f, C32 = T.wrap32_c;
             const bool wrap_ok = T.wrap32_ok != 0;
@@ -1255,11 +1353,13 @@
             for (int i = 0; i < FB_K; i++) if (i < nv) dr[(jb + i) & dmask] = x[i];
         } else
         {
-            const float a = P.deemph_alpha;
+            const float a = inv.deemph_alpha;
             const DecayW dw = load_decay(&dtab, DEC_DEEMPH, lane);
             float Ll = 0.f, Lr = 0.f;
-#pragma unroll
-            for (int i = 0; i < FB_K; i++) { Ll = (x[i].x - Ll) * a + Ll; Lr = (x[i].y - Lr) * a + Lr; }
+            SB_IF_ACTIVE {
+#pragma unroll
+                for (int i = 0; i < FB_K; i++) { Ll = (x[i].x - Ll) * a + Ll; Lr = (x[i].y - Lr) * a + Lr; }
+            }
             SB_FT(30);
             float yl, yr;
             {
@@ -1277,24 +1377,31 @@
             float2 *dr = B.dring + (size_t)ch * (dmask + 1);
             const int jb = (int)((G.J0 + seg0 + j0) & dmask);
             float el = 0.f, er_ = 0.f;
-#pragma unroll
-            for (int i = 0; i < FB_K; i++) {
-                yl = (x[i].x - yl) * a + yl;
-                yr = (x[i].y - yr) * a + yr;
-                if (i < nv) dr[(jb + i) & dmask] = make_float2(yl, yr);
-                if (i == il) { el = yl; er_ = yr; }
+            SB_IF_ACTIVE {
+#pragma unroll
+                for (int i = 0; i < FB_K; i++) {
+                    yl = (x[i].x - yl) * a + yl;
+                    yr = (x[i].y - yr) * a + yr;
+                    if (i < nv) dr[(jb + i) & dmask] = make_float2(yl, yr);
+                    if (i == il) { el = yl; er_ = yr; }
+                }
             }
             if (owner) { cy.de_l = el; cy.de_r = er_; }
         }
         SB_FT(32);
         SB_ARGS_FRESH(); SB_TICK1(7);
         }
+#undef SNAP_HERE
+#undef SB_IF_ACTIVE
     };
     for (int seg0 = 0; seg0 < nj; seg0 += FB_W) {
-        const bool fast = (nj - seg0 >= FB_W) && !((unsigned)(jx - seg0) < (unsigned)FB_W) && (callJ0 + seg0 >= 2);
-        const bool exact = PART != 2 && (P.pll_seq == 1 || (P.pll_seq == 0 && stereo_possible && !newton_ok_next) || afc_big_next);
-        if (fast) { if (exact) segment(std::true_type{}, std::true_type{}, seg0); else segment(std::true_type{}, std::false_type{}, seg0); }
-        else { if (exact) segment(std::false_type{}, std::true_type{}, seg0); else segment(std::false_type{}, std::false_type{}, seg0); }
+        const SegChoice sc = stageb_segment_form(nj, seg0, jx, callJ0, tail_fast);
+        using Full = std::integral_constant<int, 4>; using Half = std::integral_constant<int, 2>; using General = std::integral_constant<int, 0>;
+        const int pll_seq = inv_i(inv.pll_seq);
+        const bool exact = PART != 2 && (pll_seq == 1 || (pll_seq == 0 && stereo_possible && !newton_ok_next) || afc_big_next);
+        if (sc.form == SegForm::FULL_FAST) { if (exact) segment(Full{}, std::true_type{}, seg0, sc.snapshot); else segment(Full{}, std::false_type{}, seg0, sc.snapshot); }
+        else if (sc.form == SegForm::HALF_FAST) { if (exact) segment(Half{}, std::true_type{}, seg0, sc.snapshot); else segment(Half{}, std::false_type{}, seg0, sc.snapshot); }
+        else { if (exact) segment(General{}, std::true_type{}, seg0, sc.snapshot); else segment(General{}, std::false_type{}, seg0, sc.snapshot); }
     }
     __syncthreads();
     if (PART != 1 && threadIdx.x == 0) {
```
